# silvanmelchior/CBF-SSM

Measured on AMD Instinct MI355X. Metric: ELBO steps/sec, higher is better.
Workload: dtype f64; 1 GPU; C3-Sarcos train step: M=100 T=250 B=256/GPU S=20 dim_x=14 dim_u=7 dim_y=7 recog_len=16; mode=train, global_batch=256, seq_len=250, particles=20, parallelism=dp1

## Files before the change

cbf-ssm_amd/cbfssm/hip/lib.py:

```python
import ctypes as C
import os

_HERE = os.path.dirname(os.path.abspath(__file__))
LIB_PATH = os.environ.get('CBFSSM_HIP_LIB') or os.path.normpath(os.path.join(_HERE, '..', '..', 'lib', 'libcbfssm_hip.so'))

SCAL_SIGMA2, SCAL_LOGDET, SCAL_KLZ, SCAL_INFO, SCAL_COND, SCAL_JITTER, SCAL_COUNT = 0, 1, 2, 3, 4, 5, 16
GP_FORM_DENSE, GP_FORM_TRI = 0, 1
JITTER = 1e-8

SYMBOLS = (
    'cbfssm_last_error', 'cbfssm_version', 'cbfssm_gp_pack_layout', 'cbfssm_kmm_chol_f64', 'cbfssm_gp_prepare_f64',
    'cbfssm_gp_predict_f64', 'cbfssm_backward_pass_partials', 'cbfssm_backward_pass_f64',
    'cbfssm_forward_pass_partials', 'cbfssm_forward_pass_f64', 'cbfssm_loglik_moments_f64',
    'cbfssm_elbo_combine_f64', 'cbfssm_rev_workgroups', 'cbfssm_bwd_schedule', 'cbfssm_forward_pass_bwd_f64',
    'cbfssm_backward_pass_bwd_f64', 'cbfssm_reduce_partials_f64', 'cbfssm_gp_prepare2_f64', 'cbfssm_bwd_segments', 'cbfssm_forward_pass_bwd_ex_f64',
    'cbfssm_backward_pass_bwd_ex_f64', 'cbfssm_half_forward_pass_f64', 'cbfssm_half_forward_pass_bwd_f64',
    'cbfssm_saved_a2_elems', 'cbfssm_param_layout_init', 'cbfssm_constrain_f64', 'cbfssm_train_tail_work_elems',
    'cbfssm_train_tail_f64', 'cbfssm_train_tail_g_f64', 'cbfssm_train_tail_half_work_elems', 'cbfssm_train_tail_half_f64', 'cbfssm_gru_recog_param_elems', 'cbfssm_gru_recog_act_elems', 'cbfssm_gru_recog_f64', 'cbfssm_gru_recog_bwd_f64',
    'cbfssm_conv_recog_param_elems', 'cbfssm_conv_recog_f32', 'cbfssm_conv_recog_bwd_f32', 'cbfssm_adam_step_f64', 'cbfssm_loglik_partials', 'cbfssm_data_tail_f64', 'cbfssm_stash_contract_work_elems', 'cbfssm_stash_contract_f64',
    'cbfssm_cholesky_f64', 'cbfssm_rbf_k_f64', 'cbfssm_gp_predict_fullq_work_elems', 'cbfssm_gp_predict_fullq_f64',
    'cbfssm_pack_f32_elems', 'cbfssm_gp_pack_f32', 'cbfssm_gp_pack_bf16', 'cbfssm_gp_predict_f32', 'cbfssm_backward_pass_f32', 'cbfssm_forward_pass_f32',
    'cbfssm_saved_a2_f32_elems', 'cbfssm_half_forward_pass_f32', 'cbfssm_half_forward_pass_bwd_f32', 'cbfssm_rev32_slab_elems', 'cbfssm_normal_f64', 'cbfssm_philox4x32_10_u32', 'cbfssm_forward_pass_bwd_f32', 'cbfssm_backward_pass_bwd_f32',
    'cbfssm_input_adjoint_fwd_elems', 'cbfssm_input_adjoint_bwd_elems', 'cbfssm_input_adjoint_obs_elems',
    'cbfssm_forward_pass_bwd_in_f64', 'cbfssm_backward_pass_bwd_in_f64', 'cbfssm_input_grads_f64',
    'cbfssm_gp_predict_bwd_workgroups', 'cbfssm_gp_predict_bwd_work_elems', 'cbfssm_gp_predict_bwd_f64', 'cbfssm_gp_tail_f64',
    'cbfssm_gp_rollout_partials', 'cbfssm_gp_rollout_f64', 'cbfssm_gp_rollout_bwd_workgroups', 'cbfssm_gp_rollout_bwd_work_elems',
    'cbfssm_gp_rollout_bwd_f64',
    'cbfssm_gp_filter_partials', 'cbfssm_gp_filter_f64', 'cbfssm_gp_filter_bwd_workgroups', 'cbfssm_gp_filter_bwd_work_elems',
    'cbfssm_gp_filter_bwd_f64',
    'cbfssm_rigid_filter_partials', 'cbfssm_rigid_filter_f64', 'cbfssm_rigid_filter_bwd_f64',
    'cbfssm_gru_recog_bwd_in_f64', 'cbfssm_conv_recog_bwd_in_f32', 'cbfssm_half_forward_pass_bwd_in_f64',
    'cbfssm_half_input_grads_f64',
)


class ParamLayout(C.Structure):
    _fields_ = [('off', C.c_int64 * 12), ('total', C.c_int64)] + [(n, C.c_int32) for n in ('M', 'D', 'dim_x', 'dim_y')]


class PackLayout(C.Structure):
    _fields_ = [(n, C.c_int64) for n in ('total', 'Bp', 'Zp', 'cz', 'muA', 's2A', 'invl', 'scal', 'Kmm', 'L', 'Kinv',
                                          'Linvt', 'Zs', 'muB', 's2B', 'ZT', 'rev_slab', 'work', 'Wp', 'WTp')] + \
               [(n, C.c_int32) for n in ('M', 'D', 'Do', 'NBLK', 'DK', 'Mp', 'Dp', 'KS', 'JB', 'rev_stash', 'gp_form',
                                         'reserved')]


class Problem(C.Structure):
    _fields_ = [(n, C.c_int32) for n in ('B', 'S', 'T', 'dim_x', 'dim_u', 'dim_y', 'M', 'recog_len', 'condition',
                                          'half', 'group0', 'ngroups')] + [('k_factor', C.c_double)]


class RigidBody(C.Structure):
    _fields_ = [('mass_inv', C.c_double), ('inertia_inv', C.c_double * 3), ('gravity', C.c_double * 3), ('dt', C.c_double)]


class CbfssmHipError(RuntimeError):
    pass


_lib = None


def load():
    global _lib
    if _lib is not None:
        return _lib
    import torch
    if not os.path.exists(LIB_PATH):
        raise CbfssmHipError('HIP extension not built: %s is missing (run __graft_entry__.build() / make -C '
                             'cbf-ssm_amd/csrc). There is no fallback path.' % LIB_PATH)
    lib = C.CDLL(LIB_PATH)
    vp, ip, i64, dbl = C.c_void_p, C.c_int, C.c_int64, C.c_double
    lib.cbfssm_last_error.restype = C.c_char_p
    lib.cbfssm_last_error.argtypes = []
    lib.cbfssm_version.restype = ip
    lib.cbfssm_gp_pack_layout.argtypes = [ip, ip, ip, C.POINTER(PackLayout)]
    lib.cbfssm_kmm_chol_f64.argtypes = [ip, ip, vp, vp, vp, dbl, vp, vp, vp, vp, vp]
    lib.cbfssm_gp_prepare_f64.argtypes = [C.POINTER(PackLayout), vp, vp, vp, vp, vp, dbl, vp, vp]
    lib.cbfssm_gp_prepare2_f64.argtypes = ([C.POINTER(PackLayout)] + [vp] * 6) * 2 + [dbl, vp]
    lib.cbfssm_gp_predict_f64.argtypes = [C.POINTER(PackLayout), vp, vp, i64, vp, vp, vp]
    lib.cbfssm_backward_pass_partials.restype = i64
    lib.cbfssm_backward_pass_partials.argtypes = [C.POINTER(Problem)]
    lib.cbfssm_backward_pass_f64.argtypes = [C.POINTER(Problem), C.POINTER(PackLayout)] + [vp] * 12
    lib.cbfssm_forward_pass_partials.restype = i64
    lib.cbfssm_loglik_partials.restype = i64
    lib.cbfssm_loglik_partials.argtypes = [C.POINTER(Problem)]
    lib.cbfssm_param_layout_init.argtypes = [ip, ip, ip, ip, C.POINTER(ParamLayout)]
    lib.cbfssm_constrain_f64.argtypes = [C.POINTER(ParamLayout), vp, vp, vp]
    lib.cbfssm_train_tail_work_elems.restype = i64
    lib.cbfssm_train_tail_work_elems.argtypes = [C.POINTER(PackLayout), C.POINTER(PackLayout)]
    lib.cbfssm_train_tail_f64.argtypes = ([C.POINTER(ParamLayout), C.POINTER(PackLayout), vp, C.POINTER(PackLayout), vp, vp,
                                          vp, vp, i64, vp, vp, vp, vp, vp])
    lib.cbfssm_train_tail_g_f64.argtypes = ([C.POINTER(ParamLayout), C.POINTER(PackLayout), vp, C.POINTER(PackLayout), vp, vp,
                                            vp, vp, i64, ip, vp, vp, vp, vp, vp])
    lib.cbfssm_train_tail_half_work_elems.restype = i64
    lib.cbfssm_train_tail_half_work_elems.argtypes = [C.POINTER(PackLayout)]
    lib.cbfssm_train_tail_half_f64.argtypes = [C.POINTER(PackLayout), vp, vp, ip, vp, vp, i64, ip, ip, vp, vp, vp, vp, vp]
    lib.cbfssm_gru_recog_param_elems.restype = i64
    lib.cbfssm_gru_recog_param_elems.argtypes = [ip, ip, ip]
    lib.cbfssm_gru_recog_act_elems.restype = i64
    lib.cbfssm_gru_recog_act_elems.argtypes = [ip, ip]
    lib.cbfssm_gru_recog_f64.argtypes = [ip, ip, ip, ip, ip, ip, vp, vp, vp, vp, vp, vp]
    lib.cbfssm_gru_recog_bwd_f64.argtypes = [ip, ip, ip, ip, ip, ip, vp, vp, vp, vp, vp, vp, vp]
    lib.cbfssm_conv_recog_param_elems.restype = i64
    lib.cbfssm_conv_recog_param_elems.argtypes = [ip, ip, ip, ip]
    lib.cbfssm_conv_recog_f32.argtypes = [ip, ip, ip, ip, ip, ip, vp, vp, vp, vp, vp]
    lib.cbfssm_conv_recog_bwd_f32.argtypes = [ip, ip, ip, ip, ip, ip, vp, vp, vp, vp, vp, vp]
    lib.cbfssm_stash_contract_work_elems.restype = i64
    lib.cbfssm_stash_contract_work_elems.argtypes = [C.POINTER(PackLayout), i64]
    lib.cbfssm_stash_contract_f64.argtypes = [C.POINTER(PackLayout), vp, vp, i64, vp, vp, vp]
    lib.cbfssm_data_tail_f64.argtypes = [C.POINTER(Problem), vp, vp, vp, dbl, vp, vp]
    lib.cbfssm_adam_step_f64.argtypes = [i64, vp, vp, vp, vp, vp, dbl, dbl, dbl, dbl, vp]
    lib.cbfssm_saved_a2_elems.restype = i64
    lib.cbfssm_saved_a2_elems.argtypes = [C.POINTER(Problem), C.POINTER(PackLayout), ip]
    lib.cbfssm_forward_pass_partials.argtypes = [C.POINTER(Problem)]
    lib.cbfssm_forward_pass_f64.argtypes = [C.POINTER(Problem), C.POINTER(PackLayout)] + [vp] * 12
    lib.cbfssm_loglik_moments_f64.argtypes = [C.POINTER(Problem)] + [vp] * 9
    lib.cbfssm_elbo_combine_f64.argtypes = [C.POINTER(Problem), dbl, dbl, vp, i64, vp, i64, vp, i64, vp, vp, vp, vp]
    lib.cbfssm_rev_workgroups.restype = i64
    lib.cbfssm_rev_workgroups.argtypes = [C.POINTER(Problem), ip]
    lib.cbfssm_bwd_schedule.restype = ip
    lib.cbfssm_bwd_schedule.argtypes = [C.POINTER(Problem), ip] + [C.POINTER(C.c_int)] * 3
    lib.cbfssm_forward_pass_bwd_f64.argtypes = [C.POINTER(Problem), C.POINTER(PackLayout)] + [vp] * 10 + [dbl, vp, vp, vp]
    lib.cbfssm_backward_pass_bwd_f64.argtypes = [C.POINTER(Problem), C.POINTER(PackLayout)] + [vp] * 10 + [dbl, vp, vp]
    lib.cbfssm_bwd_segments.argtypes = [C.POINTER(Problem)]
    lib.cbfssm_forward_pass_bwd_ex_f64.argtypes = ([C.POINTER(Problem), C.POINTER(PackLayout)] + [vp] * 10 + [dbl, vp, vp, ip, ip, vp, vp, vp, i64, vp])
    lib.cbfssm_backward_pass_bwd_ex_f64.argtypes = ([C.POINTER(Problem), C.POINTER(PackLayout)] + [vp] * 10 + [dbl, vp, ip, ip, ip, vp, vp, i64, vp])
    lib.cbfssm_half_forward_pass_f64.argtypes = [C.POINTER(Problem), C.POINTER(PackLayout)] + [vp] * 12
    lib.cbfssm_half_forward_pass_bwd_f64.argtypes = ([C.POINTER(Problem), C.POINTER(PackLayout)] + [vp] * 9 + [dbl, vp, vp, ip, ip, vp, vp, vp, i64, vp])
    lib.cbfssm_reduce_partials_f64.argtypes = [vp, i64, i64, vp, vp]
    lib.cbfssm_cholesky_f64.argtypes = [ip, vp, dbl, vp, vp, vp, vp]
    lib.cbfssm_rbf_k_f64.argtypes = [ip, ip, ip, vp, vp, vp, vp, vp, vp]
    lib.cbfssm_gp_predict_fullq_work_elems.restype = i64
    lib.cbfssm_gp_predict_fullq_work_elems.argtypes = [C.POINTER(PackLayout), i64]
    lib.cbfssm_gp_predict_fullq_f64.argtypes = [C.POINTER(PackLayout), vp, vp, vp, i64, vp, vp, vp, vp]
    lib.cbfssm_pack_f32_elems.restype = i64
    lib.cbfssm_pack_f32_elems.argtypes = [C.POINTER(PackLayout)]
    lib.cbfssm_gp_pack_f32.argtypes = [C.POINTER(PackLayout), vp, vp, vp]
    lib.cbfssm_gp_pack_bf16.argtypes = [C.POINTER(PackLayout), vp, vp, vp]
    lib.cbfssm_gp_predict_f32.argtypes = [C.POINTER(PackLayout), vp, vp, i64, vp, vp, vp]
    lib.cbfssm_backward_pass_f32.argtypes = [C.POINTER(Problem), C.POINTER(PackLayout)] + [vp] * 12
    lib.cbfssm_forward_pass_f32.argtypes = [C.POINTER(Problem), C.POINTER(PackLayout)] + [vp] * 12
    lib.cbfssm_half_forward_pass_f32.argtypes = [C.POINTER(Problem), C.POINTER(PackLayout)] + [vp] * 12
    lib.cbfssm_half_forward_pass_bwd_f32.argtypes = [C.POINTER(Problem), C.POINTER(PackLayout)] + [vp] * 9 + [dbl, vp, vp, vp]
    lib.cbfssm_saved_a2_f32_elems.restype = i64
    lib.cbfssm_normal_f64.argtypes = [C.c_uint64, C.c_uint64, i64, vp, vp]
    lib.cbfssm_philox4x32_10_u32.argtypes = [C.c_uint64, C.c_uint64, i64, vp, vp]
    lib.cbfssm_saved_a2_f32_elems.argtypes = [C.POINTER(Problem), C.POINTER(PackLayout), ip]
    lib.cbfssm_rev32_slab_elems.restype = i64
    lib.cbfssm_rev32_slab_elems.argtypes = [C.POINTER(PackLayout)]
    lib.cbfssm_forward_pass_bwd_f32.argtypes = [C.POINTER(Problem), C.POINTER(PackLayout)] + [vp] * 10 + [dbl, vp, vp, vp]
    lib.cbfssm_backward_pass_bwd_f32.argtypes = [C.POINTER(Problem), C.POINTER(PackLayout)] + [vp] * 10 + [dbl, vp, vp]
    for name in ('cbfssm_input_adjoint_fwd_elems', 'cbfssm_input_adjoint_bwd_elems', 'cbfssm_input_adjoint_obs_elems'):
        getattr(lib, name).restype = i64
        getattr(lib, name).argtypes = [C.POINTER(Problem)]
    lib.cbfssm_forward_pass_bwd_in_f64.argtypes = ([C.POINTER(Problem), C.POINTER(PackLayout)] + [vp] * 10 + [dbl, vp, vp, ip, ip, vp, vp, vp, i64, vp, vp, vp])
    lib.cbfssm_backward_pass_bwd_in_f64.argtypes = ([C.POINTER(Problem), C.POINTER(PackLayout)] + [vp] * 10 + [dbl, vp, ip, ip, ip, vp, vp, i64, vp, vp])
    lib.cbfssm_input_grads_f64.argtypes = [C.POINTER(Problem), C.POINTER(PackLayout), vp, C.POINTER(PackLayout), vp] + [vp] * 6 + [dbl, vp, vp, vp]
    for name in ('cbfssm_gp_predict_bwd_workgroups', 'cbfssm_gp_predict_bwd_work_elems'):
        getattr(lib, name).restype = i64
        getattr(lib, name).argtypes = [C.POINTER(PackLayout), i64]
    lib.cbfssm_gp_predict_bwd_f64.argtypes = [C.POINTER(PackLayout), vp, vp, i64, vp, vp, vp, vp, vp, vp, vp]
    lib.cbfssm_gp_tail_f64.argtypes = [C.POINTER(PackLayout), vp, vp, vp, i64, dbl, vp, vp, vp, vp, vp]
    for name in ('cbfssm_gp_rollout_partials', 'cbfssm_gp_rollout_bwd_workgroups'):
        getattr(lib, name).restype = i64
        getattr(lib, name).argtypes = [C.POINTER(PackLayout), i64]
    lib.cbfssm_gp_rollout_bwd_work_elems.restype = i64
    lib.cbfssm_gp_rollout_bwd_work_elems.argtypes = [C.POINTER(PackLayout), i64, i64]
    lib.cbfssm_gp_rollout_f64.argtypes = [C.POINTER(PackLayout), vp, vp, vp, vp, vp, i64, i64, ip, vp, vp, vp, vp]
    lib.cbfssm_gp_rollout_bwd_f64.argtypes = [C.POINTER(PackLayout)] + [vp] * 8 + [i64, i64, ip] + [vp] * 6
    for name in ('cbfssm_gp_filter_partials', 'cbfssm_gp_filter_bwd_workgroups'):
        getattr(lib, name).restype = i64
        getattr(lib, name).argtypes = [C.POINTER(PackLayout), i64]
    lib.cbfssm_gp_filter_bwd_work_elems.restype = i64
    lib.cbfssm_gp_filter_bwd_work_elems.argtypes = [C.POINTER(PackLayout), i64, i64]
    lib.cbfssm_gp_filter_f64.argtypes = [C.POINTER(PackLayout)] + [vp] * 8 + [dbl, i64, i64, ip] + [vp] * 5
    lib.cbfssm_gp_filter_bwd_f64.argtypes = [C.POINTER(PackLayout)] + [vp] * 7 + [dbl] + [vp] * 5 + [i64, i64, ip] + [vp] * 7
    lib.cbfssm_rigid_filter_partials.restype = i64
    lib.cbfssm_rigid_filter_partials.argtypes = [i64]
    lib.cbfssm_rigid_filter_f64.argtypes = [C.POINTER(RigidBody)] + [vp] * 6 + [i64, i64] + [vp] * 3
    lib.cbfssm_rigid_filter_bwd_f64.argtypes = [C.POINTER(RigidBody)] + [vp] * 9 + [i64, i64] + [vp] * 5
    lib.cbfssm_gru_recog_bwd_in_f64.argtypes = [ip, ip, ip, ip, ip, ip, vp, vp, vp, vp, vp, vp, vp, vp]
    lib.cbfssm_conv_recog_bwd_in_f32.argtypes = [ip, ip, ip, ip, ip, ip, vp, vp, vp, vp, vp, vp, vp]
    lib.cbfssm_half_forward_pass_bwd_in_f64.argtypes = ([C.POINTER(Problem), C.POINTER(PackLayout)] + [vp] * 9 +
                                                        [dbl, vp, vp, ip, ip, vp, vp, vp, i64, vp, vp, vp])
    lib.cbfssm_half_input_grads_f64.argtypes = [C.POINTER(Problem), C.POINTER(PackLayout)] + [vp] * 8 + [ip, dbl, vp, vp, vp]
    for name in SYMBOLS:
        fn = getattr(lib, name)
        if name.endswith('_elems'):
            assert fn.restype is i64, name
            continue
        if fn.restype is C.c_int or name.endswith('_f64') or name.endswith('_f32') or name.endswith('_bf16') or name in ('cbfssm_gp_pack_layout', 'cbfssm_bwd_segments',
                                                                        'cbfssm_param_layout_init'):
            fn.restype = ip
    _lib = lib
    return lib


def param_layout(M, dim_x, dim_u, dim_y):
    pl = ParamLayout()
    check(load().cbfssm_param_layout_init(int(M), int(dim_x), int(dim_u), int(dim_y), C.byref(pl)), 'cbfssm_param_layout_init')
    return pl


def check(rc, what):
    if rc != 0:
        msg = load().cbfssm_last_error().decode('utf-8', 'replace')
        raise CbfssmHipError('%s failed (rc=%d): %s' % (what, rc, msg))


def rigid_body(mass_inv, inertia_inv, gravity, dt):
    rb = RigidBody()
    rb.mass_inv, rb.dt = float(mass_inv), float(dt)
# ... 18 lines not shown
```

cbf-ssm_amd/cbfssm/hip/ops.py:

```python
import ctypes as C
import os
import torch

from . import lib as _l


def _ptr(t):
    if t is None:
        return None
    assert t.is_cuda and t.dtype == torch.float64 and t.is_contiguous(), 'need contiguous float64 CUDA tensor'
    return C.c_void_p(t.data_ptr())


def _stream():
    return C.c_void_p(torch.cuda.current_stream().cuda_stream)


def _f64(t, device):
    return torch.as_tensor(t, dtype=torch.float64, device=device).contiguous()


F32_FORM_COND = 1e3


# ... 167 lines not shown


def as_btsd(x_tnd, B, S):
    T, N, d = x_tnd.shape
    return x_tnd.view(T, B, S, d).permute(1, 0, 2, 3)


def a2s_budget_bytes(device):
    cap = os.environ.get('CBFSSM_A2S_MAX_GB')
    if cap is not None:
        return float(cap) * 2 ** 30
    return 0.75 * torch.cuda.mem_get_info(torch.device(device))[0]


class TilePool:

    def __init__(self, device):
        self.device = torch.device(device)
        self.bufs = None
        self.retired = []
        self.budget = None
        self.log = []

    def get(self, n_f, n_b, reserve=0.0):
        import warnings
        if self.bufs is not None and self.bufs[0].numel() >= n_f and (n_b == 0 or (self.bufs[1] is not None and
                                                                                  self.bufs[1].numel() >= n_b)):
            return self.bufs[0][:max(n_f, 1)], (self.bufs[1][:max(n_b, 1)] if n_b else None)
        if self.budget is None:
            self.budget = a2s_budget_bytes(self.device)
        have = 0 if self.bufs is None else 8.0 * (self.bufs[0].numel() + (self.bufs[1].numel() if self.bufs[1] is not None else 0))
        need = 8.0 * (n_f + n_b)
        free_now = torch.cuda.mem_get_info(self.device)[0]
        held = float(self.bytes())
        if held + need > self.budget or need + reserve > 0.9 * free_now:
            msg = ('saved A2 tiles of this shape need %.2f GB, over the budget of %.2f GB (CBFSSM_A2S_MAX_GB): its adjoint '
                   'recomputes A2 (slower, same numbers)' % (need / 2 ** 30, self.budget / 2 ** 30))
            self.log.append(msg)
            warnings.warn(msg)
            return None, None
        if self.bufs is not None:
            msg = ('saved-A2 pool grows from %.2f to %.2f GB for a larger shape; the old buffers stay allocated for the '
                   'graphs captured on them' % (have / 2 ** 30, need / 2 ** 30))
            self.log.append(msg)
            warnings.warn(msg)
            self.retired.append(self.bufs)
        f = dict(dtype=torch.float64, device=self.device)
        self.bufs = (torch.zeros(max(n_f, 1), **f), torch.zeros(max(n_b, 1), **f) if n_b else None)
        return self.bufs[0][:max(n_f, 1)], (self.bufs[1][:max(n_b, 1)] if n_b else None)

    def bytes(self):
        tot = 0
        for pair in ([self.bufs] if self.bufs is not None else []) + self.retired:
            tot += 8 * (pair[0].numel() + (pair[1].numel() if pair[1] is not None else 0))
        return tot


class ElboWorkspace:

    def __init__(self, prob, device, keep_h=False, packs=None, pool=None):
        p = prob
        N, T = p.B * p.S, p.T
        dob = p.dim_x - p.dim_y
        f = dict(dtype=torch.float64, device=device)
        lib = _l.load()
        self.n_ent = int(lib.cbfssm_backward_pass_partials(C.byref(p)))
        self.n_kl = int(lib.cbfssm_forward_pass_partials(C.byref(p)))
        self.y2 = torch.zeros(T, N, dob, **f)
        self.h_all = torch.zeros(2, T, N, dob, **f) if keep_h else None
        self.fmv_b = torch.zeros(2, T, N, dob, 2, **f) if keep_h else None
        self.fmv_f = torch.zeros(max(T - 1, 0), N, p.dim_x, 2, **f) if keep_h else None
        self.a2s_f = self.a2s_b = None
        if keep_h and packs is not None:
            n_f = int(lib.cbfssm_saved_a2_elems(C.byref(p), C.byref(packs[0].layout), 0))
            n_b = int(lib.cbfssm_saved_a2_elems(C.byref(p), C.byref(packs[1].layout), 1)) if packs[1] is not None else 0
            if pool is None:
                pool = TilePool(device)
            reserve = 8.0 * T * N * (3 * p.dim_x + 8 * dob) + 2.0 * 2 ** 30
            self.a2s_f, self.a2s_b = pool.get(n_f, n_b, reserve)
        self.x = torch.zeros(T, N, p.dim_x, **f)
        self.ent_part = torch.zeros(self.n_ent, **f)
        self.kl_part = torch.zeros(self.n_kl, **f)
        self.ll_part = torch.zeros(int(lib.cbfssm_loglik_partials(C.byref(p))), **f)
        self.pred_mean = torch.zeros(p.B, T, p.dim_y, **f)
        self.pred_var = torch.zeros(p.B, T, p.dim_y, **f)
        self.int_mean = torch.zeros(p.B, T, p.dim_x, **f)
        self.int_var = torch.zeros(p.B, T, p.dim_x, **f)
        self.out = torch.zeros(8, **f)


def reduce_partials(gpart, slab, n, out, st):
    lib = _l.load()
    _l.check(lib.cbfssm_reduce_partials_f64(_ptr(gpart), slab, n, _ptr(out), st), 'cbfssm_reduce_partials_f64')


class TimeLoops:

    def __init__(self, prob, ws, pack_f, pack_b, var_x, var_y, u, y, eps_f, hid_b=None, eps_b=None, x0=None,
                 cL=0.0, cE=0.0, f32=False, bf16=False):
        self.prob, self.ws, self.pack_f, self.pack_b = prob, ws, pack_f, pack_b
        self.var_x, self.var_y, self.u, self.y, self.x0, self.eps_f, self.hid_b, self.eps_b = \
            var_x, var_y, u, y, x0, eps_f, hid_b, eps_b
        self.cL, self.cE, self.f32, self.bf16 = cL, cE, f32, bf16
        self.in_bufs = None

    def cast_f32(self):
        for pk in (self.pack_b, self.pack_f):
            if self.f32 and pk is not None:
                pk.pack_f32(self.bf16)

    def _gp(self, pack):
        return C.c_void_p(pack.buf32.data_ptr()) if self.f32 else _ptr(pack.buf)

    def _check(self, rc, name):
        _l.check(rc, 'cbfssm_%s_%s' % (name, 'f32' if self.f32 else 'f64'))

    def _fwd_args(self, q, *mid):
        ws = self.ws
        return ((C.byref(q), C.byref(self.pack_f.layout), self._gp(self.pack_f), _ptr(self.var_x), _ptr(self.var_y),
                 _ptr(self.u), _ptr(self.y)) + tuple(_ptr(t) for t in mid) +
                (_ptr(self.eps_f) if self.eps_f.numel() else None, _ptr(ws.x), _ptr(ws.fmv_f), _ptr(ws.a2s_f)))

    def _bwd_args(self, q):
        return (C.byref(q), C.byref(self.pack_b.layout), self._gp(self.pack_b), _ptr(self.var_x), _ptr(self.u),
                _ptr(self.y), _ptr(self.hid_b), _ptr(self.eps_b))

    def backward_pass(self, q, st):
        lib, ws = _l.load(), self.ws
        a = self._bwd_args(q) + (_ptr(ws.y2), _ptr(ws.h_all), _ptr(ws.fmv_b), _ptr(ws.a2s_b), _ptr(ws.ent_part), st)
        self._check(lib.cbfssm_backward_pass_f32(*a) if self.f32 else lib.cbfssm_backward_pass_f64(*a), 'backward_pass')

    def forward_pass(self, q, st):
        lib = _l.load()
        a = self._fwd_args(q, self.ws.y2) + (_ptr(self.ws.kl_part), st)
        self._check(lib.cbfssm_forward_pass_f32(*a) if self.f32 else lib.cbfssm_forward_pass_f64(*a), 'forward_pass')

    def forward_pass_bwd(self, q, st, chunk=None):
        lib, ws = _l.load(), self.ws
        a = self._fwd_args(q, ws.y2) + (self.cL, _ptr(ws.gy2), _ptr(ws.gpart_f))
        if self.in_bufs is not None:
            t_hi, t_lo, sa, sk, cols = chunk or (q.T - 2, 0, None, None, 0)
            _l.check(lib.cbfssm_forward_pass_bwd_in_f64(*a, t_hi, t_lo, _ptr(ws.gx_carry) if chunk else None, _ptr(sa), _ptr(sk),
                                                        cols, _ptr(self.in_bufs[0]), _ptr(self.in_bufs[2]), st),
                     'cbfssm_forward_pass_bwd_in_f64')
        elif chunk is None:
            self._check(lib.cbfssm_forward_pass_bwd_f32(*a, st) if self.f32 else lib.cbfssm_forward_pass_bwd_f64(*a, st),
                        'forward_pass_bwd')
        else:
            t_hi, t_lo, sa, sk, cols = chunk
            _l.check(lib.cbfssm_forward_pass_bwd_ex_f64(*a, t_hi, t_lo, _ptr(ws.gx_carry), _ptr(sa), _ptr(sk), cols, st),
                     'cbfssm_forward_pass_bwd_ex_f64')

    def backward_pass_bwd(self, q, st, chunk=None):
        lib, ws = _l.load(), self.ws
        a = self._bwd_args(q) + (_ptr(ws.h_all), _ptr(ws.fmv_b), _ptr(ws.a2s_b), _ptr(ws.gy2), self.cE, _ptr(ws.gpart_b))
        if self.in_bufs is not None:
            if chunk is None:
                nchunk = 0
                chunk = (0, int(lib.cbfssm_bwd_segments(C.byref(q))), None, None, 0)
            else:
                nchunk = 1
            seg0, seg1, sa, sk, cols = chunk
            _l.check(lib.cbfssm_backward_pass_bwd_in_f64(*a, seg0, seg1, nchunk, _ptr(sa), _ptr(sk), cols,
                                                         _ptr(self.in_bufs[1]), st), 'cbfssm_backward_pass_bwd_in_f64')
        elif chunk is None:
            self._check(lib.cbfssm_backward_pass_bwd_f32(*a, st) if self.f32 else lib.cbfssm_backward_pass_bwd_f64(*a, st),
                        'backward_pass_bwd')
        else:
            seg0, seg1, sa, sk, cols = chunk
            _l.check(lib.cbfssm_backward_pass_bwd_ex_f64(*a, seg0, seg1, 1, _ptr(sa), _ptr(sk), cols, st),
                     'cbfssm_backward_pass_bwd_ex_f64')

    def input_grads(self, grad_u, grad_y, st):
        ws, (gin_f, gin_b, gyo) = self.ws, self.in_bufs
        _l.check(_l.load().cbfssm_input_grads_f64(C.byref(self.prob), C.byref(self.pack_f.layout), _ptr(self.pack_f.buf),
                                                  C.byref(self.pack_b.layout), _ptr(self.pack_b.buf), _ptr(self.var_y),
                                                  _ptr(self.y), _ptr(ws.x), _ptr(gin_f), _ptr(gin_b), _ptr(gyo), self.cL,
                                                  _ptr(grad_u), _ptr(grad_y), st), 'cbfssm_input_grads_f64')

    def half_forward_pass(self, q, st):
        lib = _l.load()
        a = self._fwd_args(q, self.x0) + (_ptr(self.ws.kl_part), st)
        self._check(lib.cbfssm_half_forward_pass_f32(*a) if self.f32 else lib.cbfssm_half_forward_pass_f64(*a),
                    'half_forward_pass')

    def half_forward_pass_bwd(self, q, st, chunk=None):
        lib, ws = _l.load(), self.ws
        a = self._fwd_args(q) + (self.cL, _ptr(ws.gx0), _ptr(ws.gpart_f))
        if self.f32:
            rc = lib.cbfssm_half_forward_pass_bwd_f32(*a, st)
        else:
            t_hi, t_lo, sa, sk, cols = chunk or (q.T - 2, 0, None, None, 0)
            r = (t_hi, t_lo, _ptr(ws.gx_carry) if chunk else None, _ptr(sa), _ptr(sk), cols)
            if self.in_bufs is not None:
                _l.check(lib.cbfssm_half_forward_pass_bwd_in_f64(*a, *r, _ptr(self.in_bufs[0]), _ptr(self.in_bufs[2]), st),
                         'cbfssm_half_forward_pass_bwd_in_f64')
                return
            rc = lib.cbfssm_half_forward_pass_bwd_f64(*a, *r, st)
        self._check(rc, 'half_forward_pass_bwd')

    def half_input_grads(self, gx0, gwin, recog_len, grad_u, grad_y, st):
        ws, (gin_f, _, gyo) = self.ws, self.in_bufs
        _l.check(_l.load().cbfssm_half_input_grads_f64(C.byref(self.prob), C.byref(self.pack_f.layout), _ptr(self.pack_f.buf),
                                                       _ptr(self.var_y), _ptr(self.y), _ptr(ws.x), _ptr(gin_f), _ptr(gyo),
                                                       _ptr(gx0), _ptr(gwin), int(recog_len), self.cL, _ptr(grad_u),
                                                       _ptr(grad_y), st), 'cbfssm_half_input_grads_f64')

    def elbo_tail(self, lf0, lf1, st, kl_pack=None):
        lib, ws, pb = _l.load(), self.ws, C.byref(self.prob)
        _l.check(lib.cbfssm_loglik_moments_f64(pb, _ptr(self.var_y), _ptr(self.y), _ptr(ws.x), _ptr(ws.ll_part),
                                               _ptr(ws.pred_mean), _ptr(ws.pred_var), _ptr(ws.int_mean),
                                               _ptr(ws.int_var), st), 'cbfssm_loglik_moments_f64')
        b = self.pack_b is not None
        _l.check(lib.cbfssm_elbo_combine_f64(pb, float(lf0), float(lf1), _ptr(ws.ll_part), ws.ll_part.numel(),
                                             _ptr(ws.kl_part), ws.kl_part.numel(), _ptr(ws.ent_part) if b else None,
                                             ws.ent_part.numel() if b else 0, _ptr((kl_pack or self.pack_f).scal),
                                             _ptr(self.pack_b.scal) if b else None, _ptr(ws.out), st),
                 'cbfssm_elbo_combine_f64')


def elbo_forward(lp, loss_factors):
    prob, st = lp.prob, _stream()
    N = prob.B * prob.S
    assert lp.u.shape == (prob.B, prob.T, prob.dim_u) and lp.y.shape == (prob.B, prob.T, prob.dim_y)
    assert lp.hid_b.numel() == 2 * prob.T * N and lp.eps_b.numel() == 2 * prob.T * N
    assert lp.eps_f.numel() == (prob.T - 1) * N
    lp.cast_f32()
    lp.backward_pass(prob, st)
    lp.forward_pass(prob, st)
    lp.elbo_tail(loss_factors[0], loss_factors[1], st)
    return lp.ws


def tf_forward(x):
    return torch.nn.functional.softplus(x, beta=1.0, threshold=1e9) + 1e-10


class HipElbo:

    def __init__(self, config, device, dtype='float64'):
        self.config = config
        self.device = torch.device(device)
        assert dtype in ('float64', 'float32', 'bfloat16')
        self.f32 = dtype in ('float32', 'bfloat16')
        self.bf16 = dtype == 'bfloat16'
        self.dim_u, self.dim_y, self.dim_x = config['ds'].dim_u, config['ds'].dim_y, config['dim_x']
        self.M, self.S = config['ind_pnt_num'], config['samples']
        D = self.dim_x + self.dim_u
        mode = gp_form_mode(config) if not self.f32 else gp_form_mode_f32(config, self.bf16)
        self.pack_f = GPPack(self.M, D, self.dim_x, self.device, mode)
        self.pack_b = GPPack(self.M, D, self.dim_x - self.dim_y, self.device, mode)
        if self.f32:
            self.pack_f.cond_threshold = self.pack_b.cond_threshold = min(self.pack_f.cond_threshold, F32_FORM_COND)
        self._ws = {}

    def gp_form(self):
        return self.pack_f.gp_form() + '/' + self.pack_b.gp_form()

    def prepare(self, params):
        p = {k: _f64(v, self.device) for k, v in params.items()}
        args = [(p[g + '.zeta_pos'], tf_forward(p[g + '.lengthscales_unc']), tf_forward(p[g + '.variance_unc']),
                 p[g + '.zeta_mean'], tf_forward(p[g + '.zeta_var_unc'])) for g in 'fb']
        prepare_pair(self.pack_f, args[0], self.pack_b, args[1])
        for pk in (self.pack_f, self.pack_b):
            pk.update_form(blocking=True)
        self.var_x = tf_forward(p['var_x_unc']).contiguous()
        self.var_y = tf_forward(p['var_y_unc']).contiguous()

    def problem(self, B, T, condition):
        c = self.config
        return _l.make_problem(B, self.S, T, self.dim_x, self.dim_u, self.dim_y, self.M, c['recog_len'],
                               c['k_factor'], condition)

    def run(self, u, y, noise, condition=True, keep_h=False):
        u, y = _f64(u, self.device), _f64(y, self.device)
        B, T = u.shape[0], u.shape[1]
        prob = self.problem(B, T, condition)
        key = (B, T, keep_h)
        if key not in self._ws:
            self._ws[key] = ElboWorkspace(prob, self.device, keep_h)
        ws = self._ws[key]
        hid_b, eps_b, eps_f = (_f64(noise[k], self.device) for k in ('hid_b', 'eps_b', 'eps_f'))
        return elbo_forward(TimeLoops(prob, ws, self.pack_f, self.pack_b, self.var_x, self.var_y, u, y, eps_f, hid_b, eps_b,
                                      f32=self.f32, bf16=self.bf16), self.config['loss_factors'])


class NoisePipeline:

    def __init__(self, device, generator=None, with_backward=True):
        self.device = torch.device(device)
        self.gen = generator
        self.with_backward = with_backward
        self.stream = torch.cuda.Stream(device=self.device)
        self._bufs = {}
        self._ready = {}
        self.use_lib = not os.environ.get('CBFSSM_TORCH_NOISE')
        self.seed = int(generator.initial_seed()) & (2 ** 64 - 1) if generator is not None else int.from_bytes(os.urandom(8), 'little')
        self.offset = 0

    def _numel(self, T, N):
        return (4 * T * N if self.with_backward else 0) + (T - 1) * N

    def _fill(self, key, idx):
        buf = self._bufs[key][idx]
        cur = torch.cuda.current_stream(self.device)
        self.stream.wait_stream(cur)
        with torch.cuda.stream(self.stream):
            if self.use_lib:
                rc = _l.load().cbfssm_normal_f64(self.seed, self.offset, buf.numel(), _ptr(buf),
                                                 C.c_void_p(self.stream.cuda_stream))
                _l.check(rc, 'cbfssm_normal_f64')
                self.offset += buf.numel()
            else:
# ... 20 lines not shown
```

cbf-ssm_amd/cbfssm/hip/train.py:

```python
import ctypes as C
import math
import os
import torch

from . import lib as _l
from . import ops
from .ops import _ptr, _stream, _f64, tf_forward, GPPack
from .dist_utils import all_reduce_sum

PARAM_NAMES = (
    'f.zeta_pos', 'f.zeta_mean', 'f.zeta_var_unc', 'f.variance_unc', 'f.lengthscales_unc',
    'b.zeta_pos', 'b.zeta_mean', 'b.zeta_var_unc', 'b.variance_unc', 'b.lengthscales_unc',
    'var_x_unc', 'var_y_unc',
)
LOG2PI = math.log(2.0 * math.pi)


class FlatDict(dict):
    flat = None


def _flat_views(flat, pl, dim_u):
    M, D, dx, dy = pl.M, pl.D, pl.dim_x, pl.dim_y
    shapes = []
# ... 197 lines not shown
        else:
            loss = out[6].clone()
            terms = {'loglik': out[0], 'kl_x': out[1], 'entropy': out[2], 'kl_z_f': out[3], 'kl_z_b': out[4],
                     'info': out[7]}
        self.last_ws = ws
        return loss, terms, ws

    def _prepare(self, params, u, y, condition):
        cfg = self.config
        u, y = _f64(u, self.device), _f64(y, self.device)
        prob = _l.make_problem(u.shape[0], self.S, u.shape[1], self.dim_x, self.dim_u, self.dim_y, self.M,
                               cfg['recog_len'], cfg['k_factor'], condition)
        pflat = self._flat(params)
        p, c = self._constrained_flat(pflat)
        ops.prepare_pair(self.pack_f, (p['f.zeta_pos'], c['f.ls'], c['f.var'], p['f.zeta_mean'], c['f.zvar']),
                         self.pack_b, (p['b.zeta_pos'], c['b.ls'], c['b.var'], p['b.zeta_mean'], c['b.zvar']))
        return u, y, prob, pflat, p, c

    def _workspace(self, prob):
        key = (prob.B, prob.T)
        if key not in self._ws:
            ws = ops.ElboWorkspace(prob, self.device, keep_h=True, packs=None if self.f32 else (self.pack_f, self.pack_b),
                                   pool=self.tile_pool)
            lib = _l.load()
            n_f = int(lib.cbfssm_rev_workgroups(C.byref(prob), 0))
            n_b = int(lib.cbfssm_rev_workgroups(C.byref(prob), 1))
            f = dict(dtype=torch.float64, device=self.device)
            ws.gy2 = torch.zeros_like(ws.y2)
            if self.f32:
                if not os.environ.get('CBFSSM_F32_NO_TILES'):
                    na_f = (int(lib.cbfssm_saved_a2_f32_elems(C.byref(prob), C.byref(self.pack_f.layout), 0)) + 1) // 2
                    na_b = (int(lib.cbfssm_saved_a2_f32_elems(C.byref(prob), C.byref(self.pack_b.layout), 1)) + 1) // 2
                    assert na_f >= 0 and na_b > 0, 'record count'
                    reserve = 8.0 * prob.T * prob.B * prob.S * (3 * prob.dim_x + 8 * self.dob) + 2.0 * 2 ** 30
                    ws.a2s_f, ws.a2s_b = self.tile_pool.get(max(na_f, 1), na_b, reserve)
                sf, sb = self.slab32_f, self.slab32_b
            else:
                if self.stash:
                    n_b = 2 * n_f
                    ws.gx_carry = torch.zeros(prob.B * prob.S, prob.dim_x, **f)
                sf, sb = self.slab_f, self.slab_b
            ws.gpart_f = torch.zeros((n_f + 32) * sf, **f)
            ws.gpart_b = torch.zeros((n_b + 32) * sb, **f)
            ws.n_f, ws.n_b = n_f, n_b
            self._ws[key] = ws
        return self._ws[key]

    def loss_and_grads(self, params, u, y, noise, condition=True, weight=1.0, local=False, input_grads=False):
        s = self._grads_local(params, u, y, noise, condition, input_grads=input_grads)
        if not local:
            self._grads_collective(s, weight)
        return self._grads_finish(s)

    def _grads_collective(self, s, weight=1.0):
        if self.dist is not None:
            if weight != 1.0:
                self.red.mul_(float(weight))
            all_reduce_sum(self.red, self.dist)

    def _need_input_grads(self):
        need_input_grads(self.f32, self.dist)

    def _input_buffers(self, prob, ws):
        if getattr(ws, 'in_bufs', None) is None:
            lib = _l.load()
            f = dict(dtype=torch.float64, device=self.device)
            n = [int(fn(C.byref(prob))) for fn in (lib.cbfssm_input_adjoint_fwd_elems, lib.cbfssm_input_adjoint_bwd_elems,
                                                   lib.cbfssm_input_adjoint_obs_elems)]
            assert min(n) >= 0, n
            ws.in_bufs = tuple(torch.zeros(max(k, 1), **f) for k in n)
            ws.grad_u = torch.zeros(prob.B, prob.T, prob.dim_u, **f)
            ws.grad_y = torch.zeros(prob.B, prob.T, prob.dim_y, **f)
        return ws.in_bufs

    def _grads_local(self, params, u, y, noise, condition=True, input_grads=False):
        self._need_adjoint()
        if input_grads:
            self._need_input_grads()
        u, y, prob, pflat, p, c = self._prepare(params, u, y, condition)
        self.last_ws = ws = self._workspace(prob)
        lp = self._loops(prob, ws, c, u, y, noise)
        if input_grads:
            lp.in_bufs = self._input_buffers(prob, ws)
        self._elbo_forward(lp)
        if self.stash and not self.f32:
            gB_f, gB_b = self._adjoint_stash(lp, self.red)
        else:
            gB_f, gB_b = self._adjoint(lp, self.red)
        if input_grads:
            lp.input_grads(ws.grad_u, ws.grad_y, _stream())
        sf, sb = self.slab_f, self.slab_b
        tail = self.red[sf + sb:sf + sb + self.ntail]
        _l.check(_l.load().cbfssm_data_tail_f64(C.byref(prob), _ptr(c['var_y']), _ptr(ws.ll_part), _ptr(ws.out), lp.cL,
                                          _ptr(tail), _stream()), 'cbfssm_data_tail_f64')
        return dict(ws=ws, p=p, c=c, pflat=pflat, gB_f=gB_f, gB_b=gB_b, cL=lp.cL, cE=lp.cE, input_grads=bool(input_grads))

    def _grads_finish(self, s):
        lib = _l.load()
        st = _stream()
        ws, p, c, pflat, gB_f, gB_b, cL, cE = (s[k] for k in ('ws', 'p', 'c', 'pflat', 'gB_f', 'gB_b', 'cL', 'cE'))
        red = self.red
        sf, sb = self.slab_f, self.slab_b
        tail = red[sf + sb:sf + sb + self.ntail]
        loglik, kl_x, entropy = tail[0], tail[1], tail[2]
        kl_z_f, kl_z_b = self.pack_f.scal[_l.SCAL_KLZ], self.pack_b.scal[_l.SCAL_KLZ]
        if self.dist is not None:
            loss = -(loglik * cL - kl_x * cL + entropy * cE - kl_z_f - kl_z_b)
        else:
            loss = ws.out[6].clone()
        terms = {'loglik': loglik, 'kl_x': kl_x, 'entropy': entropy, 'kl_z_f': kl_z_f, 'kl_z_b': kl_z_b,
                 'info': ws.out[7]}
        if self.fused_tail:
            rc = lib.cbfssm_train_tail_g_f64(C.byref(self.pl), C.byref(self.pack_f.layout), _ptr(self.pack_f.buf),
                                             C.byref(self.pack_b.layout), _ptr(self.pack_b.buf), _ptr(red), _ptr(gB_f),
                                             _ptr(gB_b), 0, g_mode(self.f32, self.pack_f.layout), _ptr(pflat),
                                             _ptr(self.cflat), _ptr(self.tail_work), _ptr(self.gflat), st)
            _l.check(rc, 'cbfssm_train_tail_g_f64')
            grads = _flat_views(self.gflat, self.pl, self.dim_u)
        else:
            grads = self._grads_tensor_library(p, c, red, tail, gB_f, gB_b)
        if s.get('input_grads'):
            grads['u'], grads['y'] = ws.grad_u, ws.grad_y
        return loss, grads, terms

    def _grads_tensor_library(self, p, c, red, tail, gB_f, gB_b):
        dev = self.device
        sf, sb = self.slab_f, self.slab_b
        grads = {}
        gvx = torch.zeros(self.dim_x, dtype=torch.float64, device=dev)
        gvy = torch.zeros(self.dim_x, dtype=torch.float64, device=dev)
        if self.f32:
            gB_f, gB_b = kgk_image(self.pack_f, red[:sf], gB_f), kgk_image(self.pack_b, red[sf:sf + sb], gB_b)
        for g, pack, slab, Do, gBx in (('f', self.pack_f, red[:sf], self.dim_x, gB_f),
                                       ('b', self.pack_b, red[sf:sf + sb], self.dob, gB_b)):
            gz, gmu, gs2, gvar, gls, small = _gp_adjoint(pack, slab, p[g + '.zeta_pos'], c[g + '.ls'], c[g + '.var'],
                                                         p[g + '.zeta_mean'], c[g + '.zvar'], Do, not self.stash, gBx)
            grads.update(gp_unc_grads(g + '.', p, gz, gmu, gs2, gvar, gls))
            gvx[:Do] += small[0:Do]
            if g == 'f':
                gvy += small[16:16 + self.dim_x]
        gvy[:self.dim_y] += tail[3:]
        grads['var_x_unc'] = gvx * torch.sigmoid(p['var_x_unc'])
        grads['var_y_unc'] = gvy * torch.sigmoid(p['var_y_unc'])
        return grads

    def _split(self, prob, adjoint=True):
        if (self.stash and adjoint) or os.environ.get('CBFSSM_NO_SPLIT'):
            return None
        groups = (prob.B * prob.S + 15) // 16
        force = os.environ.get('CBFSSM_SPLIT_MAIN')
        if force:
            return (int(force), groups - int(force)) if 0 < int(force) < groups else None
        ncu = torch.cuda.get_device_properties(self.device).multi_processor_count
        if groups <= ncu or groups % ncu == 0:
            return None
        main = (groups // ncu) * ncu
        return main, groups - main

    def _sub_problem(self, prob, g0, ng):
        q = _l.Problem()
        C.memmove(C.byref(q), C.byref(prob), C.sizeof(_l.Problem))
        q.group0, q.ngroups = int(g0), int(ng)
        return q

    def _side_stream(self):
        if getattr(self, '_s1', None) is None:
            self._s1 = torch.cuda.Stream(device=self.device)
        return self._s1

    def _loops(self, prob, ws, c, u, y, noise):
        hid_b, eps_b, eps_f = (_f64(noise[k], self.device) for k in ('hid_b', 'eps_b', 'eps_f'))
        lf = self.config['loss_factors']
        return ops.TimeLoops(prob, ws, self.pack_f, self.pack_b, c['var_x'], c['var_y'], u, y, eps_f, hid_b, eps_b,
                             cL=float(lf[0]) / self.S, cE=float(lf[1]) / self.S, f32=self.f32)

    def _two_streams(self, prob, split):
        main, rest = split
        s0, s1 = torch.cuda.current_stream(), self._side_stream()
        return (self._sub_problem(prob, 0, main), self._sub_problem(prob, main, rest), s0, s1,
                C.c_void_p(s0.cuda_stream), C.c_void_p(s1.cuda_stream))

    def _elbo_forward(self, lp):
        lf = self.config['loss_factors']
        split = self._split(lp.prob, adjoint=False)
        if split is None:
            ops.elbo_forward(lp, lf)
            return
        p_main, p_rest, s0, s1, st0, st1 = self._two_streams(lp.prob, split)
        lp.cast_f32()
        e0 = torch.cuda.Event()
        e0.record(s0)
        lp.backward_pass(p_rest, st0)
        lp.forward_pass(p_rest, st0)
        s1.wait_event(e0)
        lp.backward_pass(p_main, st1)
        e1 = torch.cuda.Event()
        e1.record(s1)
        s0.wait_event(e1)
        lp.forward_pass(p_main, st0)
        lp.elbo_tail(lf[0], lf[1], st0)

    def _adjoint(self, lp, red):
        ws, st = lp.ws, _stream()
        sf, sb = self.slab_f, self.slab_b
        split = self._split(lp.prob, adjoint=False)
        if split is None:
            lp.forward_pass_bwd(lp.prob, st)
            lp.backward_pass_bwd(lp.prob, st)
        else:
            p_main, p_rest, s0, s1, st0, st1 = self._two_streams(lp.prob, split)
            lp.forward_pass_bwd(p_main, st0)
            e2 = torch.cuda.Event()
            e2.record(s0)
            lp.forward_pass_bwd(p_rest, st0)
            s1.wait_event(e2)
            lp.backward_pass_bwd(p_main, st1)
            e3 = torch.cuda.Event()
            e3.record(s1)
            lp.backward_pass_bwd(p_rest, st0)
            s0.wait_event(e3)
        if not self.repack32:
            assert not self.f32 or (self.slab32_f, self.slab32_b) == (sf, sb)
            ops.reduce_partials(ws.gpart_f, sf, ws.n_f, red[:sf], st)
            ops.reduce_partials(ws.gpart_b, sb, ws.n_b, red[sf:sf + sb], st)
            return None, None
        if self._tmp32 is None:
            self._tmp32 = torch.zeros(self.slab32_f + self.slab32_b, dtype=torch.float64, device=self.device)
        tf, tb = self._tmp32[:self.slab32_f], self._tmp32[self.slab32_f:]
        ops.reduce_partials(ws.gpart_f, self.slab32_f, ws.n_f, tf, st)
        ops.reduce_partials(ws.gpart_b, self.slab32_b, ws.n_b, tb, st)
        o = self.nred
        img_f, img_b = red[o:o + self.nimg_f], red[o + self.nimg_f:o + self.nimg_f + self.nimg_b]
        repack_f32(tf, red[:sf], img_f, self.pack_f.layout.NBLK)
        repack_f32(tb, red[sf:sf + sb], img_b, self.pack_b.layout.NBLK)
        return img_f, img_b

    def _adjoint_stash(self, lp, red):
        prob, ws = lp.prob, lp.ws
        dev = self.device
        f = dict(dtype=torch.float64, device=dev)
        Mp = self.pack_f.layout.Mp
        T, N = prob.T, prob.B * prob.S
        groups = (N + 15) // 16
        R = prob.recog_len
        P = 2 * R
        cols_f = max(groups * 16, self.stash_bytes // (4 * Mp * 8))
        cols_b = max(groups * 16 * 2 * P, self.stash_bytes // (4 * Mp * 8))
        if self._stash_buf is None or self._stash_buf[0].numel() < Mp * cols_f or self._stash_buf[2].numel() < Mp * cols_b:
            self._stash_buf = (torch.zeros(Mp * cols_f, **f), torch.zeros(Mp * cols_f, **f),
                               torch.zeros(Mp * cols_b, **f), torch.zeros(Mp * cols_b, **f))
        sa_f, sk_f, sa_b, sk_b = self._stash_buf
        sf, sb = self.slab_f, self.slab_b
        nseg = int(_l.load().cbfssm_bwd_segments(C.byref(prob)))
        per_b = max(1, cols_b // (groups * 2 * P * 16))
        prof = getattr(self, '_prof', None)
        overlap = not os.environ.get('CBFSSM_NO_SPLIT') and prof is None
        s0 = torch.cuda.current_stream()
        s1 = self._side_stream() if overlap else s0
        st0, st1 = C.c_void_p(s0.cuda_stream), C.c_void_p(s1.cuda_stream)
        red[:sf + sb].zero_()
        tmp_f, tmp_b = torch.zeros(max(sf, 1), **f), torch.zeros(max(sb, 1), **f)
        if getattr(self, '_contract', None) is None:
            o = self.nred
            self._contract = (StashContract(self.pack_f, dev, red[o:o + self.nimg_f]),
                              StashContract(self.pack_b, dev, red[o + self.nimg_f:o + self.nimg_f + self.nimg_b]))
        con_f, con_b = self._contract
        con_f.image.zero_()
        con_b.image.zero_()
        if overlap:
            s1.wait_stream(s0)

        def rfwd(t_hi, t_lo):
            per = max(1, cols_f // (groups * 16))
            while True:
                lo = max(t_lo, t_hi - per + 1)
                cols = groups * max(0, t_hi - lo + 1) * 16
                _timed(prof, 'forward_pass_adjoint', s0,
                       lambda: lp.forward_pass_bwd(prob, st0, (t_hi, lo, sa_f, sk_f, cols)))
                ev = torch.cuda.Event()
                ev.record(s0)

                def red_f():
                    ops.reduce_partials(ws.gpart_f, sf, groups, tmp_f[:sf], st0)
                    red[:sf] += tmp_f[:sf]
                _timed(prof, 'reductions', s0, red_f)
                if cols:
                    _timed(prof, 'stash_contraction', s0, lambda: con_f.add(sa_f, sk_f, cols, st0))
                if lo <= t_lo or t_hi < 0:
                    return ev
                t_hi = lo - 1

        def rbwd(seg0, seg1):
            cols = groups * 2 * (seg1 - seg0) * P * 16
            with torch.cuda.stream(s1):
                _timed(prof, 'backward_pass_adjoint', s1,
                       lambda: lp.backward_pass_bwd(prob, st1, (seg0, seg1, sa_b, sk_b, cols)))

                def red_b():
                    ops.reduce_partials(ws.gpart_b, sb, 2 * groups, tmp_b[:sb], st1)
                    red[sf:sf + sb] += tmp_b[:sb]
                _timed(prof, 'reductions', s1, red_b)
                _timed(prof, 'stash_contraction', s1, lambda: con_b.add(sa_b, sk_b, cols, st1))

        t_hi = T - 2
        seg1 = nseg
        done_all = (t_hi < 0)
        if done_all:
            rfwd(-1, 0)
# ... 66 lines not shown
class TFAdam:

    def __init__(self, params, lr, beta1=0.9, beta2=0.999, eps=1e-8):
        self.names = list(params.keys())
        sizes = [params[k].numel() for k in self.names]
        dev = params[self.names[0]].device
        self.flat = torch.cat([params[k].reshape(-1) for k in self.names]).to(torch.float64).contiguous()
        self.m = torch.zeros_like(self.flat)
        self.v = torch.zeros_like(self.flat)
        self.gflat = torch.zeros_like(self.flat)
        self.views, self.gviews = FlatDict(), {}
        self.views.flat = self.flat
        o = 0
        for k, n in zip(self.names, sizes):
            self.views[k] = self.flat[o:o + n].view(params[k].shape)
            self.gviews[k] = self.gflat[o:o + n].view(params[k].shape)
            o += n
        self.lr, self.b1, self.b2, self.eps = float(lr), beta1, beta2, eps
        self.t_dev = torch.zeros(1, dtype=torch.float64, device=dev)
        self._t = 0

    @property
    def t(self):
        return self._t

    @t.setter
    def t(self, value):
        self._t = int(value)
        self.t_dev.fill_(float(value))

    def step(self, grads):
        gflat = getattr(grads, 'flat', None)
        if gflat is not None and gflat.is_cuda and gflat.numel() == self.flat.numel():
            rc = _l.load().cbfssm_adam_step_f64(self.flat.numel(), _ptr(self.flat), _ptr(gflat), _ptr(self.m),
                                                _ptr(self.v), _ptr(self.t_dev), self.lr, self.b1, self.b2, self.eps,
                                                _stream())
            _l.check(rc, 'cbfssm_adam_step_f64')
            self._t += 1
            return
        for k in self.names:
            self.gviews[k].copy_(grads[k])
        self.t = self._t + 1
        g = self.gflat
        self.m.mul_(self.b1).add_(g, alpha=1 - self.b1)
        self.v.mul_(self.b2).addcmul_(g, g, value=1 - self.b2)
        lr_t = self.lr * math.sqrt(1 - self.b2 ** self.t) / (1 - self.b1 ** self.t)
        self.flat.addcdiv_(self.m, self.v.sqrt().add_(self.eps), value=-lr_t)

    def step_device(self, grads):
        for k in self.names:
            self.gviews[k].copy_(grads[k])
        self.t_dev.add_(1.0)
        self._t += 1
        g = self.gflat
        self.m.mul_(self.b1).add_(g, alpha=1 - self.b1)
        self.v.mul_(self.b2).addcmul_(g, g, value=1 - self.b2)
        b1t = torch.pow(torch.full_like(self.t_dev, self.b1), self.t_dev)
        b2t = torch.pow(torch.full_like(self.t_dev, self.b2), self.t_dev)
        lr_t = self.lr * torch.sqrt(1.0 - b2t) / (1.0 - b1t)
        self.flat.sub_(lr_t * self.m / (self.v.sqrt() + self.eps))

    def state_dict(self):
        return {'flat': self.flat.clone(), 'm': self.m.clone(), 'v': self.v.clone(), 't': self.t, 'names': self.names}

    def load_state_dict(self, sd):
        self.flat.copy_(sd['flat'])
        self.m.copy_(sd['m'])
        self.v.copy_(sd['v'])
        self.t = int(sd['t'])


class HipTrainStep:

    def __init__(self, config, params, device, dist=None, graph=None, engine=None, opt=None, dtype='float64'):
        if engine is None:
            engine = HipElboGrad(config, device, dist, dtype=dtype)
            opt = TFAdam({k: _f64(params[k], device).clone() for k in PARAM_NAMES}, config['learning_rate'])
        self.engine, self.opt = engine, opt
        self.params = self.opt.views
        if graph is None:
            graph = config.get('hip_graph', os.environ.get('CBFSSM_HIP_GRAPH', '1') != '0')
        self.use_graph = bool(graph) and not self.engine.stash
        self._graphs = {}
        self.last_ws = None

    def step(self, u, y, noise, condition=True, weight=1.0, local=False):
        if self.use_graph and not local:
            return self._graph_step(u, y, noise, condition, weight)
        loss, grads, terms = self.engine.loss_and_grads(self.params, u, y, noise, condition, weight=weight, local=local)
        self.opt.step(grads)
        self.last_terms = terms
        self.last_ws = self.engine.last_ws
        return loss

    def _graph_step(self, u, y, noise, condition, weight=1.0):
        dev = self.engine.device
        u, y = _f64(u, dev), _f64(y, dev)
        key = (tuple(u.shape), tuple(y.shape), bool(condition), self.engine.gp_forms())
        g = self._graphs.get(key)
        names = ('hid_b', 'eps_b', 'eps_f')
        if g is None:
            g = {'u': u.clone(), 'y': y.clone(), 'noise': {k: _f64(noise[k], dev).clone() for k in names}}
            cur = torch.cuda.current_stream(dev)
            side = torch.cuda.Stream(device=dev)
            side.wait_stream(cur)
            with torch.cuda.stream(side):
                self.engine.loss_and_grads(self.params, g['u'], g['y'], g['noise'], condition, local=True)
            cur.wait_stream(side)
            eng = self.engine
            front = None
            t_before = self.opt._t
            mode = 'global' if eng.dist is None else 'thread_local'
            try:
                if eng.dist is not None:
                    torch.cuda.synchronize(dev)
                    front = torch.cuda.CUDAGraph()
                    with torch.cuda.graph(front, capture_error_mode=mode):
                        state = eng._grads_local(self.params, g['u'], g['y'], g['noise'], condition)
                graph = torch.cuda.CUDAGraph()
                with torch.cuda.graph(graph, capture_error_mode=mode):
                    if front is None:
                        state = eng._grads_local(self.params, g['u'], g['y'], g['noise'], condition)
                    loss, grads, terms = eng._grads_finish(state)
                    if getattr(grads, 'flat', None) is not None:
                        self.opt.step(grads)
                    else:
                        self.opt.step_device(grads)
                    self.opt._t -= 1
            except RuntimeError as e:
                if eng.dist is None:
                    raise
                import warnings
                warnings.warn('HIP graph capture failed on this rank (%s): continuing with eager launches' % e)
                torch.cuda.synchronize(dev)
                self.opt._t = t_before
                self.use_graph = False
                return self.step(u, y, noise, condition, weight=weight)
            g.update(graph=graph, front=front, state=state, loss=loss, terms=terms, ws=state['ws'])
            self._graphs[key] = g
        else:
            g['u'].copy_(u)
            g['y'].copy_(y)
            for k in names:
                g['noise'][k].copy_(_f64(noise[k], dev))
        if g['front'] is not None:
            g['front'].replay()
            self.engine._grads_collective(g['state'], weight)
        g['graph'].replay()
        self.opt._t += 1
        self.last_terms = g['terms']
        self.last_ws = g['ws']
        return g['loss'].clone()
```

cbf-ssm_amd/csrc/cbfssm_api.hip:

```cpp
#include <hip/hip_runtime.h>
#include <cmath>
#include <cstdio>
#include <cstring>
#include <cstdarg>
#include <cstdlib>
#include <algorithm>
#include <map>
#include <mutex>
#include <vector>
#include "../../include/cbfssm_hip.h"
#include "cbfssm_inst.hpp"
#include "cbfssm_adjoint_inst.hpp"

CBF_FOR_EACH_NBLK(CBF_DECLARE)
CBF_FOR_EACH_REV_NBLK(CBF_REV_DECLARE)
CBF_FOR_EACH_REV_NBLK(CBF_REVIN_DECLARE)

namespace cbfssm {

static thread_local char g_err[512] = "";
static double* g_dbg = nullptr;

int fail(int code, const char* fmt, ...)
{
// ... 477 lines not shown
            hipError_t e = hipFuncSetAttribute(reinterpret_cast<const void*>(prepare_kernel<false>),
                                               hipFuncAttributeMaxDynamicSharedMemorySize, int(pl));
            if (e != hipSuccess) return fail(-int(e) - 1000, "prepare: %s", hipGetErrorString(e));
        }
        hipLaunchKernelGGL(prepare_kernel<false>, dim3(n), dim3(PREP_NT), pl, st, aa);
    }
    return check_launch("gp_prepare");
}

struct LlArgs {
    int B, S, T, dim_x, dim_y;
    const double* var_y;
    const double* y;
    const double* x;
    double* ll_part;
    double* pred_mean;
    double* pred_var;
    double* int_mean;
    double* int_var;
};

__global__ void loglik_moments_kernel(LlArgs a)
{
    __shared__ double sh[256];
    const int64_t idx = int64_t(blockIdx.x) * blockDim.x + threadIdx.x;
    const int64_t total = int64_t(a.B) * a.T * a.dim_x;
    double ll = 0.0;
    if (idx < total) {
        const int d = int(idx % a.dim_x);
        const int64_t tb = idx / a.dim_x;
        const int b = int(tb % a.B), t = int(tb / a.B);
        const int64_t bt = int64_t(b) * a.T + t;
        const int64_t N = int64_t(a.B) * a.S;
        const double* xp = a.x + (int64_t(t) * N + int64_t(b) * a.S) * a.dim_x + d;
        const double x0 = xp[0];
        double s1 = 0.0, s2 = 0.0;
        constexpr int CH = 19;
        int s = 1;
        for (; s + CH <= a.S; s += CH) {
            double v[CH];
#pragma unroll
            for (int j = 0; j < CH; ++j) v[j] = xp[int64_t(s + j) * a.dim_x];
#pragma unroll
            for (int j = 0; j < CH; ++j) {
                const double dv = v[j] - x0;
                s1 += dv;
                s2 += dv * dv;
            }
        }
#pragma unroll 8
        for (; s < a.S; ++s) {
            const double dv = xp[int64_t(s) * a.dim_x] - x0;
            s1 += dv;
            s2 += dv * dv;
        }
        const double m1 = s1 / a.S;
        const double mean = x0 + m1;
        const double ss = fmax(s2 - s1 * m1, 0.0);
        const double var = ss / a.S;
        if (a.int_mean) { a.int_mean[bt * a.dim_x + d] = mean; a.int_var[bt * a.dim_x + d] = var; }
        if (d < a.dim_y) {
            const double vy = a.var_y[d];
            const int64_t o = bt * a.dim_y + d;
            a.pred_mean[o] = mean;
            a.pred_var[o] = var + vy;
            const double yo = a.y[o];
            const double dm = yo - mean;
            const double sq = ss + a.S * dm * dm;
            ll = -0.5 * (sq / vy + a.S * (1.8378770664093454836 + log(vy)));
        }
    }
    sh[threadIdx.x] = ll;
    __syncthreads();
    if (int(threadIdx.x) < a.dim_y) {
        const int d = threadIdx.x;
        const int base = int((int64_t(blockIdx.x) * 256) % a.dim_x);
        double s = 0.0;
        for (int k = (d - base + a.dim_x) % a.dim_x; k < 256; k += a.dim_x) s += sh[k];
        a.ll_part[int64_t(blockIdx.x) * a.dim_y + d] = s;
    }
}

struct CombineArgs {
    const double* ll; int64_t n_ll;
    const double* kl; int64_t n_kl;
    const double* ent; int64_t n_ent;
    const double* scal_f;
    const double* scal_b;
    double lambda0, lambda1, inv_s;
    double* out;
};

__global__ __launch_bounds__(1024) void combine_kernel(CombineArgs a)
{
    __shared__ double red[16];
    const int tid = threadIdx.x;
    double s0 = 0.0, s1 = 0.0, s2 = 0.0;
    for (int64_t i = tid; i < a.n_ll; i += 1024) s0 += a.ll[i];
    for (int64_t i = tid; i < a.n_kl; i += 1024) s1 += a.kl[i];
    for (int64_t i = tid; i < a.n_ent; i += 1024) s2 += a.ent[i];
    const double loglik = block_sum(s0, red, tid, 1024);
    const double kl_x = block_sum(s1, red, tid, 1024);
    const double entropy = block_sum(s2, red, tid, 1024);
    if (tid == 0) {
        const double klf = a.scal_f[CBFSSM_SCAL_KLZ], klb = a.scal_b ? a.scal_b[CBFSSM_SCAL_KLZ] : 0.0;
        const double elbo = loglik * a.lambda0 * a.inv_s - kl_x * a.lambda0 * a.inv_s + entropy * a.lambda1 * a.inv_s
                            - klf - klb;
        a.out[0] = loglik; a.out[1] = kl_x; a.out[2] = entropy; a.out[3] = klf; a.out[4] = klb;
        a.out[5] = elbo; a.out[6] = -elbo;
        a.out[7] = fmax(a.scal_f[CBFSSM_SCAL_INFO], a.scal_b ? a.scal_b[CBFSSM_SCAL_INFO] : 0.0);
    }
}

#define RSPLIT 32
__global__ void reduce_partials_stage1(const double* gpart, int64_t slab, int nwg, double* tmp)
{
    const int64_t i = int64_t(blockIdx.x) * blockDim.x + threadIdx.x;
    if (i >= slab) return;
    const int part = blockIdx.y;
    const int per = (nwg + RSPLIT - 1) / RSPLIT;
    const int k0 = part * per, k1 = min(nwg, k0 + per);
    double s = 0.0;
    for (int k = k0; k < k1; ++k) s += gpart[int64_t(k) * slab + i];
    tmp[int64_t(part) * slab + i] = s;
}

__global__ void reduce_partials_stage2(const double* tmp, int64_t slab, double* out)
{
    const int64_t i = int64_t(blockIdx.x) * blockDim.x + threadIdx.x;
    if (i >= slab) return;
    double s = 0.0;
#pragma unroll
    for (int k = 0; k < RSPLIT; ++k) s += tmp[int64_t(k) * slab + i];
    out[i] = s;
}

struct InGradArgs {
    int B, S, T, dim_x, dim_u, dim_y;
    const double* gin_f;
    const double* gin_b;
    const double* gyo;
    const double* invl_f;
    const double* invl_b;
    const double* x;
    const double* y;
    const double* var_y;
    double cL;
    double* gu;
    double* gy;
};

__global__ void input_grads_kernel(InGradArgs a)
{
    const int64_t nu = int64_t(a.B) * a.T * a.dim_u, ny = int64_t(a.B) * a.T * a.dim_y;
    const int64_t i = int64_t(blockIdx.x) * blockDim.x + threadIdx.x;
    if (i >= nu + ny) return;
    const int64_t N = int64_t(a.B) * a.S;
    const int naux = a.dim_u + a.dim_y, dob = a.dim_x - a.dim_y;
    const bool is_u = i < nu;
    const int nd = is_u ? a.dim_u : a.dim_y;
    const int64_t e = is_u ? i : i - nu;
    const int k = int(e % nd);
    const int t = int((e / nd) % a.T);
    const int b = int(e / (int64_t(nd) * a.T));
    const int ja = is_u ? k : a.dim_u + k;
    const double* p0 = a.gin_b + ((int64_t(0) * a.T + t) * naux + ja) * N + int64_t(b) * a.S;
    const double* p1 = a.gin_b + ((int64_t(1) * a.T + t) * naux + ja) * N + int64_t(b) * a.S;
    double s0 = 0.0, s1 = 0.0;
    for (int s = 0; s < a.S; ++s) { s0 += p0[s]; s1 += p1[s]; }
    double r = a.invl_b[dob + ja] * (s0 + s1);
    if (is_u) {
        if (t < a.T - 1) {
            const double* pf = a.gin_f + (int64_t(t) * a.dim_u + k) * N + int64_t(b) * a.S;
            double sf = 0.0;
            for (int s = 0; s < a.S; ++s) sf += pf[s];
            r += a.invl_f[a.dim_x + k] * sf;
        }
        a.gu[e] = r;
    } else {
        const double* po = a.gyo + (int64_t(t) * a.dim_y + k) * N + int64_t(b) * a.S;
        const double* px = a.x + (int64_t(t) * N + int64_t(b) * a.S) * a.dim_x + k;
        const double yv = a.y[e];
        double so = 0.0, sl = 0.0;
        for (int s = 0; s < a.S; ++s) {
// ... 403 lines not shown
    PredictArgs a;
    a.pk = pack_ptrs(L, pack); a.X = X; a.npts = npts; a.D = L->D; a.Do = L->Do; a.fmean = fmean; a.fvar = fvar;
    a.tri = (L->gp_form == CBFSSM_GP_FORM_TRI);
    a.a2o = work;
    int rc = dispatch_predict(L->NBLK, L->DK, a, (hipStream_t)stream);
    if (rc) return fail(rc, "gp_predict launch failed (NBLK=%d DK=%d rc=%d)", L->NBLK, L->DK, rc);
    const size_t lds = size_t(16) * L->NBLK * 16 * sizeof(double);
    if (lds > 48 * 1024) {
        hipError_t e = hipFuncSetAttribute(reinterpret_cast<const void*>(fullq_kernel),
                                           hipFuncAttributeMaxDynamicSharedMemorySize, int(lds));
        if (e != hipSuccess) return fail(-int(e) - 1000, "fullq: %s", hipGetErrorString(e));
    }
    hipLaunchKernelGGL(fullq_kernel, dim3(unsigned((npts + 15) / 16), unsigned(L->Do)), dim3(256), lds, (hipStream_t)stream,
                       (const double*)work, q_sqrt, L->M, L->NBLK, L->Do, npts, fvar);
    return check_launch("gp_predict_fullq");
}

int64_t cbfssm_backward_pass_partials(const cbfssm_problem* p)
{
    if (!p || p->recog_len < 1) return -1;
    int n0, n1;
    bwd_segments(p, &n0, &n1);
    const int64_t groups = (int64_t(p->B) * p->S + 15) / 16;
    return groups * (n0 + n1);
}

static int save_k(const cbfssm_pack_layout* L);

int cbfssm_backward_pass_f64(const cbfssm_problem* p, const cbfssm_pack_layout* L, const double* pack_b,
                             const double* var_x, const double* u, const double* y, const double* hid_b,
                             const double* eps_b, double* y2, double* h_all, double* fmv_b, double* a2s_b,
                             double* ent_part, void* stream)
{
    int rc = check_problem(p, L, p ? p->dim_x - p->dim_y : 0);
    if (rc) return rc;
    if (p->dim_x - p->dim_y < 1) return fail(-1, "backward pass needs dim_x > dim_y (use CBFSSMHALF otherwise)");
    if (!pack_b || !var_x || !u || !y || !hid_b || !eps_b || !y2 || !ent_part) return fail(-1, "null pointer");
    PassArgs a;
    memset(&a, 0, sizeof(a));
    a.pk = pack_ptrs(L, pack_b);
    a.N = p->B * p->S; a.S = p->S; a.T = p->T; a.B = p->B;
    a.dim_x = p->dim_x; a.dim_u = p->dim_u; a.dim_y = p->dim_y; a.Do = p->dim_x - p->dim_y; a.D = L->D;
    a.recog_len = p->recog_len; a.condition = p->condition; a.k_factor = p->k_factor;
    a.var_x = var_x; a.u = u; a.y = y; a.eps = eps_b; a.hid = hid_b; a.y2_out = y2; a.h_all = h_all;
    a.part_out = ent_part;
    a.dbg = g_dbg;
    a.fmv = fmv_b;
    a.a2s = a2s_b;
    a.ksave = save_k(L);
    int n0, n1;
    bwd_segments(p, &n0, &n1);
    a.nseg0 = n0;
    a.tri = (L->gp_form == CBFSSM_GP_FORM_TRI);
    const int nc = a.tri ? 1 : pass_nc(p, MODE_BWD);
    int g0, ng, gt;
    rc = group_range(p, nc, &g0, &ng, &gt);
    if (rc) return rc;
    a.group0 = g0; a.gtotal = gt;
    dim3 grid(unsigned(ng), unsigned(n0 + n1));
    rc = dispatch_pass(L->NBLK, L->DK, MODE_BWD, a, grid, nc, (hipStream_t)stream);
    if (rc) return fail(rc, "backward_pass launch failed (NBLK=%d DK=%d rc=%d)", L->NBLK, L->DK, rc);
    return 0;
}

static int save_k(const cbfssm_pack_layout* L) { return (L->NBLK <= 7 && !getenv("CBFSSM_NO_SAVE_K")) ? 1 : 0; }

int64_t cbfssm_saved_a2_elems(const cbfssm_problem* p, const cbfssm_pack_layout* L, int backward)
{
    if (!p || !L) return -1;
    const int64_t g16 = (int64_t(p->B) * p->S + 15) / 16;
    const int64_t slots = backward ? 2 * int64_t(p->T) : (p->T > 1 ? p->T - 1 : 0);
    return slots * g16 * saved_tile_stride(L->NBLK, save_k(L));
}

int64_t cbfssm_forward_pass_partials(const cbfssm_problem* p)
{
    if (!p) return -1;
    return (int64_t(p->B) * p->S + 15) / 16;
}

static int forward_pass_impl(const cbfssm_problem* p, const cbfssm_pack_layout* L, const double* pack_f,
                             const double* var_x, const double* var_y, const double* u, const double* y,
                             const double* y2, const double* x0, const double* eps_f, double* x, double* fmv_f,
                             double* a2s_f, double* kl_part, void* stream)
{
    int rc = check_problem(p, L, p ? p->dim_x : 0);
    if (rc) return rc;
    if (!pack_f || !var_x || !var_y || !u || !y || !x || !kl_part) return fail(-1, "null pointer");
    if (p->half ? !x0 : (p->dim_x > p->dim_y && !y2)) return fail(-1, p->half ? "x0 is null" : "y2 is null");
    if (p->T > 1 && !eps_f) return fail(-1, "eps_f is null");
    PassArgs a;
    memset(&a, 0, sizeof(a));
    a.pk = pack_ptrs(L, pack_f);
    a.N = p->B * p->S; a.S = p->S; a.T = p->T; a.B = p->B;
    a.dim_x = p->dim_x; a.dim_u = p->dim_u; a.dim_y = p->dim_y; a.Do = p->dim_x; a.D = L->D;
    a.recog_len = p->recog_len; a.condition = p->condition; a.k_factor = p->k_factor;
    a.var_x = var_x; a.var_y = var_y; a.u = u; a.y = y; a.eps = eps_f; a.y2_in = y2; a.x_out = x;
    a.part_out = kl_part;
    a.dbg = g_dbg;
    a.half = p->half; a.x0 = x0;
    a.fmv = fmv_f;
    a.a2s = a2s_f;
    a.ksave = save_k(L);
    a.tri = (L->gp_form == CBFSSM_GP_FORM_TRI);
    const int nc = a.tri ? 1 : pass_nc(p, MODE_FWD);
    int g0, ng, gt;
    rc = group_range(p, nc, &g0, &ng, &gt);
    if (rc) return rc;
    a.group0 = g0; a.gtotal = gt;
    dim3 grid(unsigned(ng), 1);
    rc = dispatch_pass(L->NBLK, L->DK, MODE_FWD, a, grid, nc, (hipStream_t)stream);
    if (rc) return fail(rc, "forward_pass launch failed (NBLK=%d DK=%d rc=%d)", L->NBLK, L->DK, rc);
    return 0;
}

int cbfssm_forward_pass_f64(const cbfssm_problem* p, const cbfssm_pack_layout* L, const double* pack_f,
                            const double* var_x, const double* var_y, const double* u, const double* y,
                            const double* y2, const double* eps_f, double* x, double* fmv_f, double* a2s_f,
                            double* kl_part, void* stream)
{
    if (p && p->half) return fail(-1, "problem->half is set: use cbfssm_half_forward_pass_f64");
    return forward_pass_impl(p, L, pack_f, var_x, var_y, u, y, y2, nullptr, eps_f, x, fmv_f, a2s_f, kl_part, stream);
}

int cbfssm_half_forward_pass_f64(const cbfssm_problem* p, const cbfssm_pack_layout* L, const double* pack_f,
                                 const double* var_x, const double* var_y, const double* u, const double* y,
                                 const double* x0, const double* eps_f, double* x, double* fmv_f, double* a2s_f,
                                 double* kl_part, void* stream)
{
    if (!p || !p->half) return fail(-1, "problem->half must be 1");
    return forward_pass_impl(p, L, pack_f, var_x, var_y, u, y, nullptr, x0, eps_f, x, fmv_f, a2s_f, kl_part, stream);
}

int cbfssm_loglik_moments_f64(const cbfssm_problem* p, const double* var_y, const double* y, const double* x,
                              double* ll_part, double* pred_mean, double* pred_var, double* int_mean,
                              double* int_var, void* stream)
{
    if (!p || !var_y || !y || !x || !ll_part || !pred_mean || !pred_var) return fail(-1, "null pointer");
    if ((int_mean == nullptr) != (int_var == nullptr)) return fail(-1, "int_mean/int_var must both be given");
    LlArgs a;
    a.B = p->B; a.S = p->S; a.T = p->T; a.dim_x = p->dim_x; a.dim_y = p->dim_y;
    a.var_y = var_y; a.y = y; a.x = x; a.ll_part = ll_part; a.pred_mean = pred_mean; a.pred_var = pred_var;
    a.int_mean = int_mean; a.int_var = int_var;
    const int64_t total = int64_t(p->B) * p->T * p->dim_x;
    const int64_t nblk = (total + 255) / 256;
    hipLaunchKernelGGL(loglik_moments_kernel, dim3(unsigned(nblk)), dim3(256), 0, (hipStream_t)stream, a);
    return check_launch("loglik_moments");
}

int64_t cbfssm_loglik_partials(const cbfssm_problem* p)
{
    if (!p) return -1;
    return (int64_t(p->B) * p->T * p->dim_x + 255) / 256 * p->dim_y;
}

int cbfssm_elbo_combine_f64(const cbfssm_problem* p, double lambda0, double lambda1, const double* ll_part,
                            int64_t n_ll, const double* kl_part, int64_t n_kl, const double* ent_part, int64_t n_ent,
                            const double* scal_f, const double* scal_b, double* out, void* stream)
{
    if (!p || !scal_f || !out) return fail(-1, "null pointer");
    CombineArgs a;
    a.ll = ll_part; a.n_ll = ll_part ? n_ll : 0; a.kl = kl_part; a.n_kl = kl_part ? n_kl : 0;
    a.ent = ent_part; a.n_ent = ent_part ? n_ent : 0;
    a.scal_f = scal_f; a.scal_b = scal_b; a.lambda0 = lambda0; a.lambda1 = lambda1; a.inv_s = 1.0 / p->S;
    a.out = out;
    hipLaunchKernelGGL(combine_kernel, dim3(1), dim3(1024), 0, (hipStream_t)stream, a);
    return check_launch("elbo_combine");
}

constexpr int SCHED_UNITS = 256;
constexpr int SCHED_PER_RUN = 16;
constexpr int SCHED_PROLOGUE = 2;

struct SchedEntry { int run, t_begin, nsteps; };

static bool sched_table(int T, int R, int m, std::vector<SchedEntry>& out)
{
    const int P = 2 * R;
    out.clear();
    for (int run = 0; run < 2; ++run) {
        const int start = run * R;
        int rem = (T > start) ? (T - start + P - 1) / P : 0, pos = 0, cnt = 0;
        while (rem > 0) {
            const int c = std::min(m, std::max(1, rem / 2));
            const int tb = start + P * pos, te = std::min(T, start + P * (pos + c));
            out.push_back({run, tb, te - tb});
            pos += c; rem -= c;
            if (++cnt > SCHED_PER_RUN) return false;
        }
    }
    std::stable_sort(out.begin(), out.end(), [](const SchedEntry& x, const SchedEntry& y) { return x.nsteps > y.nsteps; });
    return true;
}

static int64_t sched_makespan(const std::vector<SchedEntry>& tab, int64_t groups)
{
    std::map<int64_t, int64_t> slots;
    slots[0] = SCHED_UNITS;
    for (const SchedEntry& e : tab) {
        int64_t left = groups;
        while (left > 0) {
            auto it = slots.begin();
            const int64_t t = it->first, take = std::min(left, it->second);
            if ((it->second -= take) == 0) slots.erase(it);
            slots[t + e.nsteps + SCHED_PROLOGUE] += take;
            left -= take;
        }
    }
    return slots.rbegin()->first;
}

static void bwd_schedule(int T, int R, int64_t n, std::vector<SchedEntry>& best)
{
    static std::mutex mu;
    static int cT = -1, cR = -1;
    static int64_t cn = -1;
    static std::vector<SchedEntry> cached;
    std::lock_guard<std::mutex> lock(mu);
    if (T != cT || R != cR || n != cn) {
        const int64_t groups = (n + 15) / 16;
        const int P = 2 * R;
        std::vector<SchedEntry> tab;
        int64_t best_t = -1;
        cached.clear();
        for (int m = std::max(1, (T + P - 1) / P); m >= 1; --m) {
            if (!sched_table(T, R, m, tab)) break;
            const int64_t t = sched_makespan(tab, groups);
            if (best_t < 0 || t < best_t) { best_t = t; cached = tab; }
        }
        cT = T; cR = R; cn = n;
    }
    best = cached;
}

static int bwd_total_segments(const cbfssm_problem* p)
{
    return (p->T - 1 + p->recog_len) / (2 * p->recog_len) + 1;
}

int cbfssm_bwd_schedule(const cbfssm_problem* p, int cap, int* run, int* t_begin, int* nsteps)
{
    if (!p || p->recog_len < 1 || p->T < 1 || p->B < 1 || p->S < 1) return fail(-1, "bad problem");
    std::vector<SchedEntry> tab;
    bwd_schedule(p->T, p->recog_len, int64_t(p->B) * p->S, tab);
    const int n = int(tab.size());
    if (run || t_begin || nsteps) {
        if (!run || !t_begin || !nsteps || cap < n) return fail(-1, "schedule has %d entries (cap %d)", n, cap);
        for (int i = 0; i < n; ++i) { run[i] = tab[i].run; t_begin[i] = tab[i].t_begin; nsteps[i] = tab[i].nsteps; }
    }
    return n;
// ... 330 lines not shown
```

cbf-ssm_amd/csrc/cbfssm_kernels.hpp:

```cpp
#pragma once
#include <hip/hip_runtime.h>
#include <stdint.h>
#include <type_traits>

namespace cbfssm {

typedef double d4 __attribute__((ext_vector_type(4)));

#define CBF_MFMA(a, b, c) __builtin_amdgcn_mfma_f64_16x16x4f64((a), (b), (c), 0, 0, 0)

__device__ __forceinline__ double fast_rcp(double x)
{
    double r = __builtin_amdgcn_rcp(x);
    r = fma(r, fma(-x, r, 1.0), r);
    return fma(r, fma(-x, r, 1.0), r);
}
__device__ __forceinline__ double fast_rsqrt(double x)
{
    double y = __builtin_amdgcn_rsq(x);
    const double hx = 0.5 * x;
    y = fma(y, fma(-hx * y, y, 0.5), y);
    return fma(y, fma(-hx * y, y, 0.5), y);
}

// ... 197 lines not shown
        "v_mfma_f64_16x16x4_f64 %[c01], v[150:151], v[166:167], %[c01]\n\t"
        "v_mfma_f64_16x16x4_f64 %[c11], v[158:159], v[166:167], %[c11]\n\t"
        "s_branch 4f\n\t"
        "3:\n"
        "s_waitcnt vmcnt(0) lgkmcnt(0)\n\t"
        "v_mfma_f64_16x16x4_f64 %[c00], v[120:121], v[136:137], %[c00]\n\t"
        "v_mfma_f64_16x16x4_f64 %[c10], v[128:129], v[136:137], %[c10]\n\t"
        "v_mfma_f64_16x16x4_f64 %[c01], v[122:123], v[138:139], %[c01]\n\t"
        "v_mfma_f64_16x16x4_f64 %[c11], v[130:131], v[138:139], %[c11]\n\t"
        "v_mfma_f64_16x16x4_f64 %[c00], v[124:125], v[140:141], %[c00]\n\t"
        "v_mfma_f64_16x16x4_f64 %[c10], v[132:133], v[140:141], %[c10]\n\t"
        "v_mfma_f64_16x16x4_f64 %[c01], v[126:127], v[142:143], %[c01]\n\t"
        "v_mfma_f64_16x16x4_f64 %[c11], v[134:135], v[142:143], %[c11]\n\t"
        "4:\n"
        "s_nop 15\n\t"
        "s_nop 2\n\t"
        : [c00] "+v"(c00), [c01] "+v"(c01), [c10] "+v"(c10), [c11] "+v"(c11), [pa0] "+v"(pa0), [pa1] "+v"(pa1),
          [pb] "+v"(ldsb), [n] "+s"(ngrp)
        : [step] "s"(step), [bs0] "n"(0 * BSTRIDE), [bs1] "n"(1 * BSTRIDE), [bs2] "n"(2 * BSTRIDE), [bs3] "n"(3 * BSTRIDE),
          [bs4] "n"(4 * BSTRIDE), [bs5] "n"(5 * BSTRIDE), [bs6] "n"(6 * BSTRIDE), [bs7] "n"(7 * BSTRIDE),
          [bs8] "n"(8 * BSTRIDE)
        : "scc", "v120", "v121", "v122", "v123", "v124", "v125", "v126", "v127", "v128", "v129", "v130", "v131", "v132", "v133", "v134", "v135", "v136", "v137", "v138", "v139", "v140", "v141", "v142", "v143", "v144", "v145", "v146", "v147", "v148", "v149", "v150", "v151", "v152", "v153", "v154", "v155", "v156", "v157", "v158", "v159", "v160", "v161", "v162", "v163", "v164", "v165", "v166", "v167");
}

struct PackPtrs {
    const double* Bp;
    const double* Zp;
    const double* cz;
    const double* muA;
    const double* s2A;
    const double* invl;
    const double* scal;
    int KSr;
    const double* Wp;
    const double* WTp;
};

typedef __attribute__((address_space(3))) int lds_int;
__device__ __forceinline__ void flag_release(int* f, int v)
{
    __hip_atomic_store((lds_int*)f, v, __ATOMIC_RELEASE, __HIP_MEMORY_SCOPE_WORKGROUP);
}
#define CBF_FLAG_TIMEOUT_SLOT 96
__device__ __forceinline__ void flag_wait(int* flags, int idx, int v)
{
    int spins = 0;
    while (__hip_atomic_load((lds_int*)(flags + idx), __ATOMIC_ACQUIRE, __HIP_MEMORY_SCOPE_WORKGROUP) < v) {
        __builtin_amdgcn_s_sleep(1);
        if (++spins > (1 << 22)) {
            __hip_atomic_store((lds_int*)(flags + CBF_FLAG_TIMEOUT_SLOT), 1, __ATOMIC_RELAXED, __HIP_MEMORY_SCOPE_WORKGROUP);
            break;
        }
    }
}

struct PassArgs {
    PackPtrs pk;
    int N, S, T, B;
    int dim_x, dim_u, dim_y;
    int Do;
    int D;
    int recog_len, condition;
    double k_factor;
    const double* var_x;
    const double* var_y;
    const double* u;
    const double* y;
    const double* eps;
    const double* hid;
    const double* y2_in;
    double* y2_out;
    double* h_all;
    double* x_out;
    double* part_out;
    int nseg0;
    double* dbg;
    int half;
    const double* x0;
    int group0, gtotal;
    double* a2s;
    double* fmv;
    int tri;
    int ksave;
};

__device__ __forceinline__ int bwd_segment(int y, int n0, int ny, int& run, int& k, bool& dead)
{
    const int n1 = ny - n0, w1 = max(0, n1 - 2);
    dead = false;
    if (y < n0 - 1) { run = 0; k = y + 1; }
    else if (y < n0 - 1 + w1) { run = 1; k = y - (n0 - 1) + 2; }
    else if (y == n0 - 1 + w1) { run = 0; k = n0; }
    else if (y == ny - 1) { run = 1; k = 1; dead = true; }
    else { run = 1; k = n1; }
    return run == 0 ? k - 1 : n0 + k - 1;
}

__host__ __device__ constexpr int saved_tile_stride(int nblk, int ksave) { return nblk * 256 * (ksave ? 2 : 1); }

struct PredictArgs {
    PackPtrs pk;
    const double* X;
    int64_t npts;
    int D, Do;
    double* fmean;
    double* fvar;
    int tri;
    double* a2o;
};

template <int NBLK, int RB, int DK, bool BREG, bool TRI = false, int KT = -1>
struct Tile {
    static constexpr int W = (NBLK + RB - 1) / RB;
    static constexpr int NT = 64 * W;
    static constexpr int MP = 16 * NBLK;
    static constexpr int KS = MP / 4;
    static constexpr bool EXACT = (KT >= 0);
    static constexpr int KSE = EXACT ? KS - KT : KS;
    static_assert(!EXACT || (BREG && KT < 4), "the trim applies to register-resident tiles, within the last row block");
    static constexpr int QPW = (4 + W - 1) / W;
    static constexpr int TRI_LDS = TRI ? MP * 16 + 64 : 0;
    static constexpr int LDS_DOUBLES = DK * 64 + MP * 16 + W * 512 + 64 + TRI_LDS;
    static constexpr int NBR = BREG ? (TRI ? KSE + 4 : KSE) : 1;
    static_assert(!(TRI && BREG) || RB == 1, "register-resident triangular operands: one row block per wave");

    __device__ __forceinline__ static int rb_of(int w, int i)
    {
        if constexpr (TRI && BREG && NBLK == 7) {
            return (w == 3) ? 6 : ((w < 3) ? 5 - w : w - 4);
        } else {
            return w * RB + i;
        }
    }
    static constexpr int EPI_LDS_N = BREG ? 0 : (LDS_DOUBLES + 2 * NBLK * 256 <= 20480 ? 2 : (LDS_DOUBLES + NBLK * 256 <= 20480 ? 1 : 0));
    static constexpr bool EPI_LDS = EPI_LDS_N > 0;
    static constexpr int EPI_LDS_DOUBLES = EPI_LDS_N * NBLK * 256;

    double Zreg[RB][DK];
    double czr[RB][4];
    double muA[RB][4];
    double s2A[RB][4];
    double Breg[BREG ? RB : 1][NBR];
    const double* Bp;
    const double* Wp;
    const double* WTp;
    const double* muAg;
    const double* s2Ag;
    int lane_;
    double sigma2;
    int KSr;
    int koff;

    template <bool WITH_EPI = true>
    __device__ __forceinline__ void load_operands(const PackPtrs& pk, int w, int l)
    {
        Bp = pk.Bp;
        Wp = pk.Wp;
        WTp = pk.WTp;
        muAg = pk.muA;
        s2Ag = pk.s2A;
        lane_ = l;
        sigma2 = pk.scal[0];
        KSr = pk.KSr;
        koff = 0;
#pragma unroll
        for (int i = 0; i < RB; ++i) {
// ... 524 lines not shown
#pragma unroll
    for (int qi = 0; qi < TT::QPW; ++qi) {
        const int q = w + qi * TT::W;
        if (q < 4) {
            double fm, fv;
            tile.gather(part, q, l, fm, fv);
            const int d = 4 * q + (l >> 4);
            const int64_t p = p0 + (l & 15);
            if (d < a.Do && p < a.npts) {
                a.fmean[p * a.Do + d] = fm;
                a.fvar[p * a.Do + d] = fv;
            }
        }
    }
}

template <int NBLK, int RB, int DK, bool BREG, int MODE, int NC, bool TRI = false, int KT = -1>
__global__ __launch_bounds__(64 * ((NBLK + RB - 1) / RB)) void pass_kernel(PassArgs a)
{
    static_assert(!TRI || NC == 1, "the two-triangular form runs one column block per workgroup");
    typedef Tile<NBLK, RB, DK, BREG, TRI, KT> TT;
    constexpr int W = TT::W, NT = TT::NT;
    constexpr int NTASK = 4 * NC;
    constexpr int QPW = (NTASK + W - 1) / W;
    constexpr int AUXR = (DK * 64 + NT - 1) / NT;
    constexpr int XS = DK * 64, KTS = TT::MP * 16, PS = W * 512;
    extern __shared__ double lds[];
    double* xq = lds;
    double* Kt = xq + NC * XS;
    double* part = Kt + NC * KTS;
    double* red = part + NC * PS;
    double* At = red + 64 + ((TT::EPI_LDS && NC == 1) ? TT::EPI_LDS_DOUBLES : 0);
    int* flag = reinterpret_cast<int*>(At + TT::MP * 16);

    const int tid = threadIdx.x, l = tid & 63, w = tid >> 6, g = l >> 4, nl = l & 15;
    const int N = a.N, S = a.S, T = a.T, Do = a.Do;
    const int naux = a.D - Do;
    const int gx = blockIdx.x + a.group0;
    const int c0 = gx * 16 * NC;
    const int G16 = (N + 15) >> 4;

    int t_first, nsteps, dir, run = 0, slot = 0;
    const int R = a.recog_len, P = 2 * R;
    if (MODE == MODE_FWD) {
        t_first = 0; nsteps = T - 1; dir = 1;
    } else {
        int k;
        bool dead;
        slot = bwd_segment(blockIdx.y, a.nseg0, gridDim.y, run, k, dead);
        const int o = run * R;
        const int hi = min(P * k - 1 - o, T - 1);
        const int lo = (k > 1) ? (P * (k - 1) - o) : 0;
        t_first = hi; nsteps = dead ? 0 : hi - lo + 1; dir = -1;
        if (nsteps <= 0) {
            if (tid == 0) {
                const int G16p = (a.N + 15) >> 4;
                for (int cq = 0; cq < NC; ++cq)
                    if (gx * NC + cq < G16p) a.part_out[slot * G16p + gx * NC + cq] = (cq == 0) ? 0.0 : 0.0;
            }
            return;
        }
    }

    TT tile;
    tile.load_operands(a.pk, w, l);
    tile.koff = a.ksave ? NBLK * 256 : 0;
    if constexpr (TT::EPI_LDS && NC == 1) {
        double* mul = red + 64;
        for (int i = tid; i < NBLK * 256; i += NT) mul[i] = a.pk.muA[i];
        tile.muAg = mul;
        if constexpr (TT::EPI_LDS_N == 2) {
            double* s2l = mul + NBLK * 256;
            for (int i = tid; i < NBLK * 256; i += NT) s2l[i] = a.pk.s2A[i];
            tile.s2Ag = s2l;
        }
    }

    double vx[QPW], vy[QPW], il[QPW];
    double hcur[QPW];
    double lin[QPW];
    LogProd lp[QPW];
    bool act[QPW], cval[QPW];
    int cc[QPW], bqv[QPW], qv[QPW], cbv[QPW];
#pragma unroll
    for (int qi = 0; qi < QPW; ++qi) {
        const int tk = w + qi * W;
        qv[qi] = tk & 3;
        cbv[qi] = (tk >> 2) < NC ? (tk >> 2) : (NC - 1);
        const int d = 4 * qv[qi] + g;
        const int cg = c0 + cbv[qi] * 16 + nl;
        cc[qi] = min(cg, N - 1);
        cval[qi] = cg < N;
        bqv[qi] = cc[qi] / S;
        act[qi] = (tk < NTASK) && (d < Do);
        const int dc = act[qi] ? d : 0;
        vx[qi] = a.var_x[dc];
        vy[qi] = (MODE == MODE_FWD) ? a.var_y[(a.half && dc >= a.dim_y) ? 0 : dc] : 0.0;
        il[qi] = a.pk.invl[dc];
        lin[qi] = 0.0;
        lp[qi].init();
        hcur[qi] = 0.0;
    }

    const double* auxp[NC][AUXR];
    int auxs[NC][AUXR];
    double auxl[NC][AUXR];
#pragma unroll
    for (int cb = 0; cb < NC; ++cb)
#pragma unroll
        for (int k2 = 0; k2 < AUXR; ++k2) {
            const int i = tid + k2 * NT, ja = i >> 4, n = i & 15;
            auxp[cb][k2] = a.pk.invl; auxs[cb][k2] = 0; auxl[cb][k2] = 0.0;
            if (i < 16 * naux) {
                const int b = min(c0 + cb * 16 + n, N - 1) / S;
                if (ja < a.dim_u) { auxp[cb][k2] = a.u + int64_t(b) * T * a.dim_u + ja; auxs[cb][k2] = a.dim_u; }
                else { auxp[cb][k2] = a.y + int64_t(b) * T * a.dim_y + (ja - a.dim_u); auxs[cb][k2] = a.dim_y; }
                auxl[cb][k2] = a.pk.invl[Do + ja];
            }
        }
    auto aux_load = [&](int cb, int k2, int t) -> double { return auxp[cb][k2][int64_t(t) * auxs[cb][k2]]; };

    for (int i = tid; i < NC * XS; i += NT) xq[i] = 0.0;
    if constexpr (TRI) {
        if (tid < 64) { flag[tid] = 0; flag[tid + 64] = 0; }
    }
    __syncthreads();
    const bool resample0 = (MODE == MODE_BWD) && (((t_first + 1 + run * R) % P) == 0);
    const int tm0 = (MODE == MODE_BWD) ? (t_first % P) : 0;
#pragma unroll
    for (int qi = 0; qi < QPW; ++qi) {
        const int d = 4 * qv[qi] + g;
        const int c = cc[qi];
        if (act[qi]) {
            double v;
            if (MODE == MODE_FWD) {
                if (a.half) v = a.x0[int64_t(bqv[qi]) * a.dim_x + d];
                else v = (d < a.dim_y) ? a.y[(int64_t(bqv[qi]) * T) * a.dim_y + d]
                                       : a.y2_in[int64_t(c) * (a.dim_x - a.dim_y) + (d - a.dim_y)];
                if (cval[qi]) a.x_out[int64_t(c) * a.dim_x + d] = v;
            } else {
                v = resample0 ? a.hid[(int64_t(run) * T + t_first) * N + c] : 0.0;
            }
            hcur[qi] = v;
            xq[cbv[qi] * XS + 64 * qv[qi] + l] = v * il[qi];
        }
    }
    double auxr[NC][AUXR];
#pragma unroll
    for (int cb = 0; cb < NC; ++cb)
#pragma unroll
        for (int k2 = 0; k2 < AUXR; ++k2) {
            const int i = tid + k2 * NT;
            if (i < 16 * naux) xq[cb * XS + 16 * Do + i] = aux_load(cb, k2, t_first) * auxl[cb][k2];
        }

    CBF_STAMP_DECL;
    CBF_STAMP_START();
    for (int step = 0; step < nsteps; ++step) {
        const int t = t_first + dir * step;
        const int tn = t + dir;
        int tmod = tm0 - step; if (tmod < 0) tmod += P;
        const int tmn = (tmod == 0) ? P - 1 : tmod - 1;
        const bool has_next = (step + 1 < nsteps);
        CBF_STAMP_BARRIER(0);

        double eps_t[QPW], ytil[QPW], hidn[QPW];
        bool resample_n = false;
        if (MODE == MODE_BWD) resample_n = has_next && (tmn + 1 + run * R == P);
#pragma unroll
        for (int qi = 0; qi < QPW; ++qi) {
            const int c = cc[qi];
            const int d = 4 * qv[qi] + g;
            ytil[qi] = 0.0; hidn[qi] = 0.0;
            if (MODE == MODE_FWD) {
                eps_t[qi] = a.eps[int64_t(t) * N + c];
                if (act[qi]) {
                    if (d < a.dim_y) ytil[qi] = a.y[(int64_t(bqv[qi]) * T + (t + 1)) * a.dim_y + d];
                    else if (!a.half) ytil[qi] = a.y2_in[(int64_t(t + 1) * N + c) * (a.dim_x - a.dim_y) + (d - a.dim_y)];
                }
            } else {
                eps_t[qi] = a.eps[(int64_t(run) * T + t) * N + c];
                if (resample_n) hidn[qi] = a.hid[(int64_t(run) * T + tn) * N + c];
            }
        }
#pragma unroll
        for (int cb = 0; cb < NC; ++cb)
#pragma unroll
            for (int k2 = 0; k2 < AUXR; ++k2) {
                const int i = tid + k2 * NT;
                auxr[cb][k2] = has_next ? aux_load(cb, k2, tn) : 0.0;
            }

        double* a2o = nullptr;
        if (a.a2s) {
            const int64_t slot = (MODE == MODE_FWD) ? int64_t(t) : (int64_t(run) * T + t);
            a2o = a.a2s + (slot * G16 + int64_t(gx) * NC) * (NBLK * 256 + tile.koff);
        }
        if constexpr (NC == 1) {
            double kr[RB][4];
            tile.phase1(xq, Kt, kr, w, l);
#pragma unroll
            for (int qi = 0; qi < QPW; ++qi) asm volatile("" : "+v"(eps_t[qi]), "+v"(ytil[qi]), "+v"(hidn[qi]));
#pragma unroll
            for (int cb = 0; cb < NC; ++cb)
#pragma unroll
                for (int k2 = 0; k2 < AUXR; ++k2) asm volatile("" : "+v"(auxr[cb][k2]));
            if constexpr (TRI) {
                if (a2o && tile.koff) {
#pragma unroll
                    for (int i = 0; i < RB; ++i) {
                        const int rb = tile.rb_of(w, i);
                        if (rb < NBLK) {
#pragma unroll
                            for (int r = 0; r < 4; ++r) a2o[tile.koff + rb * 256 + r * 64 + l] = kr[i][r];
                        }
                    }
                }
            }
            CBF_STAMP_BARRIER(1);
            if constexpr (TRI) tile.phase2_tri(Kt, At, flag, step + 1, part, w, l, a2o);
            else tile.phase2(Kt, part, kr, w, l, a2o);
        } else {
            tile.template gp_phases<NC>(xq, Kt, part, w, l, a2o, G16 - gx * NC);
        }
        CBF_STAMP_BARRIER(2);

#pragma unroll
        for (int qi = 0; qi < QPW; ++qi) {
            const int tk = w + qi * W;
            if (tk < NTASK) {
                const int q = qv[qi], cb = cbv[qi], c = cc[qi];
                double fm, fv;
                tile.gather(part + cb * PS, q, l, fm, fv);
                const int d = 4 * q + g;
                double outv = 0.0;
                if (act[qi]) {
                    const double fmean = fm + hcur[qi];
                    const double fvar = fv + vx[qi];
                    if (a.fmv && cval[qi]) {
                        const int64_t slot = (MODE == MODE_FWD) ? int64_t(t) : (int64_t(run) * T + t);
                        double* o = a.fmv + ((slot * N + c) * Do + d) * 2;
                        o[0] = fmean; o[1] = fvar;
                    }
                    if (MODE == MODE_FWD) {
                        const double vyt = vy[qi] + (a.k_factor - 1.0) * fvar;
                        const double s = vyt + fvar;
                        const double rs = fast_rcp(s);
                        const double kk = fvar * rs;
                        const double ydiff = ytil[qi] - fmean;
                        const double dm = kk * ydiff;
                        const double mu = fmean + dm;
                        const double sig = kk * vyt;
                        const bool do_cond = (a.condition || (t < R - 1)) && !(a.half && d >= a.dim_y);
                        outv = do_cond ? (mu + eps_t[qi] * (sig * fast_rsqrt(sig)))
                                       : (fmean + eps_t[qi] * (fvar * fast_rsqrt(fvar)));
                        if (do_cond && cval[qi]) {
                            lin[qi] += kk * (ydiff * ydiff * rs - 1.0);
                            lp[qi].mul(vyt * rs);
                        }
                        if (cval[qi]) a.x_out[(int64_t(t + 1) * N + c) * a.dim_x + d] = outv;
                    } else {
                        outv = fmean + eps_t[qi] * (fvar * fast_rsqrt(fvar));
                        const bool write = (run == 0) ? (tmod < R) : (tmod >= R);
                        if (cval[qi]) {
                            if (write) {
                                a.y2_out[(int64_t(t) * N + c) * Do + d] = outv;
                                lp[qi].mul(fvar);
                                lin[qi] += 1.0;
                            }
                            if (a.h_all) a.h_all[((int64_t(run) * T + t) * N + c) * Do + d] = outv;
                        }
                    }
                }
                const double hn = (MODE == MODE_BWD && resample_n) ? hidn[qi] : outv;
                hcur[qi] = act[qi] ? hn : 0.0;
                if (has_next && act[qi]) xq[cb * XS + 64 * q + l] = hn * il[qi];
            }
        }
        if (has_next) {
#pragma unroll
            for (int cb = 0; cb < NC; ++cb)
#pragma unroll
                for (int k2 = 0; k2 < AUXR; ++k2) {
                    const int i = tid + k2 * NT;
                    if (i < 16 * naux) xq[cb * XS + 16 * Do + i] = auxr[cb][k2] * auxl[cb][k2];
                }
        }
    }

    double v = 0.0;
#pragma unroll
    for (int qi = 0; qi < QPW; ++qi) {
        if (act[qi] && cval[qi]) {
            if (MODE == MODE_FWD) v += 0.5 * (lin[qi] - lp[qi].log());
            else v += 0.5 * (lin[qi] * 2.8378770664093453391 + lp[qi].log());
        }
    }
    double tot = block_sum(v, red, tid, NT);
    if constexpr (TRI) {
        if (tid == 0 && flag[CBF_FLAG_TIMEOUT_SLOT] != 0) tot = __builtin_nan("");
    }
    if (tid == 0) {
        const int G16p = (a.N + 15) >> 4;
        for (int cq = 0; cq < NC; ++cq)
            if (gx * NC + cq < G16p) a.part_out[slot * G16p + gx * NC + cq] = (cq == 0) ? tot : 0.0;
    }
#ifdef CBF_REV_STAMPS
#ifndef CBF_STAMP_WAVE_PASS
#define CBF_STAMP_WAVE_PASS (W - 1)
#endif
    if (a.dbg && l == 0 && (w == 0 || w == CBF_STAMP_WAVE_PASS)) {
        double* o = a.dbg + (int64_t(slot) * a.gtotal + gx) * 64 + (w == 0 ? 0 : 32);
        for (int i = 0; i < 7; ++i) { o[i] = double(st_c[i]); o[7 + i] = double(st_w[i]); }
        for (int i = 0; i < 12; ++i) o[14 + i] = double(st_m[i]);
    }
#endif
}

template <int NBLK, int RB, int DK, bool BREG, int MODE, int KT = -1>
__global__ __launch_bounds__(64 * ((NBLK + RB - 1) / RB)) void pass_kernel_skew(PassArgs a)
{
    typedef Tile<NBLK, RB, DK, BREG, false, KT> TT;
    constexpr int W = TT::W, NT = TT::NT;
    constexpr int QPW = TT::QPW;
    constexpr int AUXR = (DK * 64 + NT - 1) / NT;
    constexpr int XS = DK * 64, KTS = TT::MP * 16, PS = W * 512;
    extern __shared__ double lds[];
    double* xq = lds;
    double* Kt = xq + 2 * XS;
    double* part = Kt + 2 * KTS;
    double* red = part + 2 * PS;

    const int tid = threadIdx.x, l = tid & 63, w = tid >> 6, g = l >> 4, nl = l & 15;
    const int N = a.N, S = a.S, T = a.T, Do = a.Do;
    const int naux = a.D - Do;
    const int gx = blockIdx.x + a.group0;
    const int c0 = gx * 32;

    int t_first, nsteps, dir, run = 0, slot = 0;
    const int R = a.recog_len, P = 2 * R;
    if (MODE == MODE_FWD) {
        t_first = 0; nsteps = T - 1; dir = 1;
    } else {
        int k;
        bool dead;
        slot = bwd_segment(blockIdx.y, a.nseg0, gridDim.y, run, k, dead);
        const int o = run * R;
        const int hi = min(P * k - 1 - o, T - 1);
        const int lo = (k > 1) ? (P * (k - 1) - o) : 0;
        t_first = hi; nsteps = dead ? 0 : hi - lo + 1; dir = -1;
        if (nsteps <= 0) {
            if (tid == 0) {
                const int G16p = (a.N + 15) >> 4;
                for (int cq = 0; cq < 2; ++cq)
                    if (gx * 2 + cq < G16p) a.part_out[slot * G16p + gx * 2 + cq] = (cq == 0) ? 0.0 : 0.0;
            }
            return;
        }
    }

    TT tile;
    tile.load_operands(a.pk, w, l);
    tile.koff = a.ksave ? NBLK * 256 : 0;

    double vx[2][QPW], vy[2][QPW], il[2][QPW], hcur[2][QPW], lin[2][QPW];
    LogProd lp[2][QPW];
    bool act[2][QPW], cval[2];
    int cc[2], bqv[2];
#pragma unroll
    for (int c = 0; c < 2; ++c) {
        const int cg = c0 + c * 16 + nl;
        cc[c] = min(cg, N - 1);
        cval[c] = cg < N;
        bqv[c] = cc[c] / S;
        const int wq = (c == 0) ? w : (W - 1 - w);
#pragma unroll
        for (int qi = 0; qi < QPW; ++qi) {
            const int q = wq + qi * W;
            const int d = 4 * q + g;
            act[c][qi] = (q < 4) && (d < Do);
            const int dc = act[c][qi] ? d : 0;
            vx[c][qi] = a.var_x[dc];
            vy[c][qi] = (MODE == MODE_FWD) ? a.var_y[dc] : 0.0;
            il[c][qi] = a.pk.invl[dc];
            lin[c][qi] = 0.0;
            lp[c][qi].init();
            hcur[c][qi] = 0.0;
        }
    }

    const double* auxp[2][AUXR];
    int auxs[2][AUXR];
    double auxl[2][AUXR];
#pragma unroll
    for (int cb = 0; cb < 2; ++cb)
#pragma unroll
        for (int k2 = 0; k2 < AUXR; ++k2) {
            const int i = tid + k2 * NT, ja = i >> 4, n = i & 15;
            auxp[cb][k2] = a.pk.invl; auxs[cb][k2] = 0; auxl[cb][k2] = 0.0;
            if (i < 16 * naux) {
                const int b = min(c0 + cb * 16 + n, N - 1) / S;
                if (ja < a.dim_u) { auxp[cb][k2] = a.u + int64_t(b) * T * a.dim_u + ja; auxs[cb][k2] = a.dim_u; }
                else { auxp[cb][k2] = a.y + int64_t(b) * T * a.dim_y + (ja - a.dim_u); auxs[cb][k2] = a.dim_y; }
                auxl[cb][k2] = a.pk.invl[Do + ja];
            }
        }
    auto aux_load = [&](int cb, int k2, int t) -> double { return auxp[cb][k2][int64_t(t) * auxs[cb][k2]]; };

    for (int i = tid; i < 2 * XS; i += NT) xq[i] = 0.0;
    __syncthreads();
    const bool resample0 = (MODE == MODE_BWD) && (((t_first + 1 + run * R) % P) == 0);
    const int tm0 = (MODE == MODE_BWD) ? (t_first % P) : 0;
#pragma unroll
    for (int c = 0; c < 2; ++c) {
        const int wq = (c == 0) ? w : (W - 1 - w);
#pragma unroll
        for (int qi = 0; qi < QPW; ++qi) {
            const int q = wq + qi * W;
            const int d = 4 * q + g;
            if (act[c][qi]) {
                double v;
                if (MODE == MODE_FWD) {
                    v = (d < a.dim_y) ? a.y[(int64_t(bqv[c]) * T) * a.dim_y + d]
                                      : a.y2_in[int64_t(cc[c]) * (a.dim_x - a.dim_y) + (d - a.dim_y)];
                    if (cval[c]) a.x_out[int64_t(cc[c]) * a.dim_x + d] = v;
                } else {
                    v = resample0 ? a.hid[(int64_t(run) * T + t_first) * N + cc[c]] : 0.0;
                }
                hcur[c][qi] = v;
                xq[c * XS + 64 * q + l] = v * il[c][qi];
            }
        }
#pragma unroll
        for (int k2 = 0; k2 < AUXR; ++k2) {
            const int i = tid + k2 * NT;
            if (i < 16 * naux) xq[c * XS + 16 * Do + i] = aux_load(c, k2, t_first) * auxl[c][k2];
        }
    }
    __syncthreads();

    double kregA[RB][4], kregB[RB][4];

    auto phase3 = [&](auto cidx, int s) {
        constexpr int c = decltype(cidx)::value;
        const int t = t_first + dir * s;
        const int tn = t + dir;
        int tmod = tm0 - s; if (tmod < 0) tmod += P;
        const int tmn = (tmod == 0) ? P - 1 : tmod - 1;
        const bool has_next = (s + 1 < nsteps);
        const int wq = (c == 0) ? w : (W - 1 - w);
        const int cch = cc[c];
        bool resample_n = false;
        if (MODE == MODE_BWD) resample_n = has_next && (tmn + 1 + run * R == P);
        double eps_t, hidn = 0.0;
        if (MODE == MODE_FWD) eps_t = a.eps[int64_t(t) * N + cch];
        else {
            eps_t = a.eps[(int64_t(run) * T + t) * N + cch];
            if (resample_n) hidn = a.hid[(int64_t(run) * T + tn) * N + cch];
        }
        double auxn[AUXR];
#pragma unroll
        for (int k2 = 0; k2 < AUXR; ++k2) {
            const int i = tid + k2 * NT;
            auxn[k2] = has_next ? aux_load(c, k2, tn) : 0.0;
        }
#pragma unroll
        for (int qi = 0; qi < QPW; ++qi) {
            const int q = wq + qi * W;
            if (q < 4) {
                const int d = 4 * q + g;
                double ytil = 0.0;
                if (MODE == MODE_FWD && act[c][qi])
                    ytil = (d < a.dim_y) ? a.y[(int64_t(bqv[c]) * T + (t + 1)) * a.dim_y + d]
                                         : a.y2_in[(int64_t(t + 1) * N + cch) * (a.dim_x - a.dim_y) + (d - a.dim_y)];
                double fm, fv;
                tile.gather(part + c * PS, q, l, fm, fv);
                double outv = 0.0;
                if (act[c][qi]) {
                    const double fmean = fm + hcur[c][qi];
                    const double fvar = fv + vx[c][qi];
                    if (a.fmv && cval[c]) {
                        const int64_t slot = (MODE == MODE_FWD) ? int64_t(t) : (int64_t(run) * T + t);
                        double* o = a.fmv + ((slot * N + cch) * Do + d) * 2;
                        o[0] = fmean; o[1] = fvar;
                    }
                    if (MODE == MODE_FWD) {
                        const double vyt = vy[c][qi] + (a.k_factor - 1.0) * fvar;
                        const double sm = vyt + fvar;
                        const double rs = fast_rcp(sm);
                        const double kk = fvar * rs;
                        const double ydiff = ytil - fmean;
                        const double mu = fmean + kk * ydiff;
                        const double sig = kk * vyt;
                        const bool do_cond = a.condition || (t < R - 1);
                        outv = do_cond ? (mu + eps_t * (sig * fast_rsqrt(sig))) : (fmean + eps_t * (fvar * fast_rsqrt(fvar)));
                        if (do_cond && cval[c]) {
                            lin[c][qi] += kk * (ydiff * ydiff * rs - 1.0);
                            lp[c][qi].mul(vyt * rs);
                        }
                        if (cval[c]) a.x_out[(int64_t(t + 1) * N + cch) * a.dim_x + d] = outv;
                    } else {
                        outv = fmean + eps_t * (fvar * fast_rsqrt(fvar));
                        const bool write = (run == 0) ? (tmod < R) : (tmod >= R);
                        if (cval[c]) {
                            if (write) {
                                a.y2_out[(int64_t(t) * N + cch) * Do + d] = outv;
                                lp[c][qi].mul(fvar);
                                lin[c][qi] += 1.0;
                            }
                            if (a.h_all) a.h_all[((int64_t(run) * T + t) * N + cch) * Do + d] = outv;
                        }
                    }
                }
                const double hn = (MODE == MODE_BWD && resample_n) ? hidn : outv;
                hcur[c][qi] = act[c][qi] ? hn : 0.0;
                if (has_next && act[c][qi]) xq[c * XS + 64 * q + l] = hn * il[c][qi];
            }
        }
        if (has_next) {
#pragma unroll
            for (int k2 = 0; k2 < AUXR; ++k2) {
                const int i = tid + k2 * NT;
                if (i < 16 * naux) xq[c * XS + 16 * Do + i] = auxn[k2] * auxl[c][k2];
            }
        }
    };
    using I0 = std::integral_constant<int, 0>;
    using I1 = std::integral_constant<int, 1>;

    const int G16 = (N + 15) >> 4;
    auto a2slot = [&](int s, int c) -> double* {
        if (!a.a2s || 2 * gx + c >= G16) return nullptr;
        const int t = t_first + dir * s;
        const int64_t slot = (MODE == MODE_FWD) ? int64_t(t) : (int64_t(run) * T + t);
        return a.a2s + (slot * G16 + 2 * gx + c) * (NBLK * 256 + tile.koff);
    };
    tile.phase1(xq, Kt, kregA, w, l);
    __syncthreads();
    const bool hi = (w >= 4);
    for (int s = 0; s < nsteps; ++s) {
        if (hi) {
            if (s > 0) phase3(I1{}, s - 1);
            tile.phase2(Kt, part, kregA, w, l, a2slot(s, 0));
        } else {
            tile.phase2(Kt, part, kregA, w, l, a2slot(s, 0));
            if (s > 0) phase3(I1{}, s - 1);
        }
        __syncthreads();
        if (hi) {
            tile.phase1(xq + XS, Kt + KTS, kregB, w, l);
            phase3(I0{}, s);
        } else {
            phase3(I0{}, s);
            tile.phase1(xq + XS, Kt + KTS, kregB, w, l);
        }
        __syncthreads();
        if (hi) {
            tile.phase2(Kt + KTS, part + PS, kregB, w, l, a2slot(s, 1));
            if (s + 1 < nsteps) tile.phase1(xq, Kt, kregA, w, l);
        } else {
            if (s + 1 < nsteps) tile.phase1(xq, Kt, kregA, w, l);
            tile.phase2(Kt + KTS, part + PS, kregB, w, l, a2slot(s, 1));
        }
        __syncthreads();
    }
    phase3(I1{}, nsteps - 1);

    double v = 0.0;
#pragma unroll
    for (int c = 0; c < 2; ++c)
#pragma unroll
        for (int qi = 0; qi < QPW; ++qi) {
            if (act[c][qi] && cval[c]) {
                if (MODE == MODE_FWD) v += 0.5 * (lin[c][qi] - lp[c][qi].log());
                else v += 0.5 * (lin[c][qi] * 2.8378770664093453391 + lp[c][qi].log());
            }
        }
    const double tot = block_sum(v, red, tid, NT);
    if (tid == 0) {
        const int G16p = (a.N + 15) >> 4;
        for (int cq = 0; cq < 2; ++cq)
            if (gx * 2 + cq < G16p) a.part_out[slot * G16p + gx * 2 + cq] = (cq == 0) ? tot : 0.0;
    }
}

}
```

cbf-ssm_amd/csrc/cbfssm_tail.hip:

```cpp
#include <hip/hip_runtime.h>
#include <stdint.h>
#include <string.h>

#include "../../include/cbfssm_hip.h"

namespace cbfssm {

int fail(int rc, const char* fmt, ...);

struct GpTail {
    const double* slab;
    const double* gB_dense;
    int64_t gB_ld;
    const double* Kinv;
    const double* Kmm;
    const double* Zs;
    double* T;
    double* G2;
    double* dv;
    const double* scal;
    const double* zmean;
    const double* zvar;
    const double* ls;
    const double* var;
// ... 219 lines not shown
        p.g_z[idx] = gzt / p.ls[p.shared_ls ? 0 : j];
    }
    __syncthreads();
    for (int j = wv; j < D; j += NT / 64) {
        double s = 0.0;
        for (int i = l; i < M; i += 64) s += p.g_z[i * D + j] * p.Zs[i * D + j];
        for (int o = 32; o > 0; o >>= 1) s += __shfl_xor(s, o);
        if (l == 0) {
            const double sx = nd ? 0.0 : small[32 + j];
            if (p.shared_ls) glsj[j] = -(s + sx / p.ls[0]);
            else p.g_ls[j] = -(s + sx / p.ls[j]) * sigmoid(p.ls_unc[j]);
        }
    }
    if (p.shared_ls) {
        __syncthreads();
        if (tid == 0) {
            double s = 0.0;
            for (int j = 0; j < D; ++j) s += glsj[j];
            p.g_ls[0] = s * sigmoid(p.ls_unc[0]);
        }
    }
    if (tid == 0) {
        const double var = p.var[0];
        const double s96 = nd ? 0.0 : small[96], s97 = nd ? 0.0 : small[97];
        p.g_var[0] = (tot / var + s96 + s97 / var) * sigmoid(p.var_unc[0]);
    }
    for (int idx = tid; idx < M * Do; idx += NT) {
        const int i = idx / Do, d = idx - i * Do;
        const double gm0 = nd ? 0.0 : c_image(gMu, 1, i, d), gs0 = nd ? 0.0 : c_image(gS2, 1, i, d);
        p.g_mu[idx] = gm0 + p.klw * KM[idx];
        const double gs2 = gs0 + p.klw * 0.5 * ((p.Kkl ? p.Kkl : p.Kinv)[int64_t(i) * M + i] - 1.0 / p.zvar[idx]);
        p.g_s2[idx] = gs2 * sigmoid(p.zvar_unc[idx]);
    }
    if (blockIdx.x == 0 && tid < a.dim_x) {
        double gvx = small[tid];
        if (a.ngp > 1) {
            const GpTail& pb = a.gp[1];
            const double* small_b = pb.slab + 2 * pb.NBLK * 256 + (pb.stash ? 0 : pb.NBLK * pb.NBLK * 256) + pb.NBLK * pb.JB * 256;
            if (tid < pb.Do) gvx += small_b[tid];
        }
        a.g_vx[tid] = gvx * sigmoid(a.vx_unc[tid]);
        if (tid < a.n_vy) {
            double gvy = small[16 + tid];
            if (tid < a.dim_y) gvy += a.tail[3 + tid];
            a.g_vy[tid] = gvy * sigmoid(a.vy_unc[tid]);
        }
    }
}

struct ConstrainArgs {
    const double* p;
    double* c;
    int64_t off[13];
    int unc[12];
};

__global__ __launch_bounds__(256) void constrain_kernel(ConstrainArgs a)
{
    const int64_t i = int64_t(blockIdx.x) * 256 + threadIdx.x;
    if (i >= a.off[12]) return;
    int seg = 0;
#pragma unroll
    for (int s = 1; s < 12; ++s) seg += (i >= a.off[s]);
    const double x = a.p[i];
    a.c[i] = a.unc[seg] ? (fmax(x, 0.0) + log1p(exp(-fabs(x))) + 1e-10) : x;
}

__global__ __launch_bounds__(256) void data_tail_kernel(const double* ll_part, int64_t nblk, int dim_y, const double* var_y,
                                                        const double* out8, double cL, double bts, double* tail)
{
    __shared__ double red[4];
    const int tid = threadIdx.x, d = blockIdx.x;
    double s = 0.0;
    for (int64_t k = tid; k < nblk; k += 256) s += ll_part[k * dim_y + d];
    const double tot = block_sum_t(s, red, tid, 256);
    if (tid == 0) {
        const double vy = var_y[d];
        const double sq = (-2.0 * tot - bts * (1.8378770664093454836 + log(vy))) * vy;
        tail[3 + d] = -cL * 0.5 * (sq / (vy * vy) - bts / vy);
    }
    if (d == 0 && tid < 3) tail[tid] = out8[tid];
}

__global__ void adam_tick_kernel(double* t) { t[0] += 1.0; }

__global__ __launch_bounds__(256) void adam_kernel(int64_t n, double* p, const double* g, double* m, double* v, const double* t,
                                                   double lr, double b1, double b2, double eps)
{
    const int64_t i = int64_t(blockIdx.x) * 256 + threadIdx.x;
    if (i >= n) return;
    const double tt = t[0];
    const double lr_t = lr * sqrt(1.0 - pow(b2, tt)) / (1.0 - pow(b1, tt));
    const double gi = g[i];
    const double mi = b1 * m[i] + (1.0 - b1) * gi;
    const double vi = b2 * v[i] + (1.0 - b2) * gi * gi;
    m[i] = mi;
    v[i] = vi;
    p[i] -= lr_t * mi / (sqrt(vi) + eps);
}

}

namespace cbfssm {

static int one_gp_tail(const cbfssm_pack_layout* L, const double* pack, const double* pack_kl, int shared_ls, const double* slab,
                       const double* gB_dense, int64_t gB_ld, int g_mode, double klw, int dim_y, const double* pflat,
                       const double* cflat, double* work, double* gflat, void* stream, const char* what)
{
    TailArgs a;
    memset(&a, 0, sizeof(a));
    GpTail& p = a.gp[0];
    const int M = L->M, D = L->D, Do = L->Do;
    p.slab = slab;
    p.gB_dense = gB_dense; p.gB_ld = gB_ld;
    p.Kinv = pack + L->Kinv; p.Kmm = pack + L->Kmm; p.Zs = pack + L->Zs;
    double* w = work;
    p.T = w; w += int64_t(M) * (M > 48 ? M : 48);
    p.G2 = w; w += int64_t(M) * M;
    p.T2 = w; w += int64_t(M) * M;
    p.dv = w;
    p.scal = pack + L->scal;
    p.Kkl = pack_kl ? pack_kl + L->Kinv : nullptr;
    p.shared_ls = shared_ls ? 1 : 0;
    p.klw = klw; p.nodata = slab ? 0 : 1;
    const int64_t o1 = int64_t(M) * D, o2 = o1 + int64_t(M) * Do, o3 = o2 + int64_t(M) * Do, o4 = o3 + 1,
                  o5 = o4 + (shared_ls ? 1 : D), o6 = o5 + Do;
    p.zmean = cflat + o1; p.zvar = cflat + o2; p.var = cflat + o3; p.ls = cflat + o4;
    p.zvar_unc = pflat + o2; p.var_unc = pflat + o3; p.ls_unc = pflat + o4;
    p.g_z = gflat; p.g_mu = gflat + o1; p.g_s2 = gflat + o2; p.g_var = gflat + o3; p.g_ls = gflat + o4;
    p.M = M; p.D = D; p.Do = Do; p.NBLK = L->NBLK; p.JB = L->JB; p.stash = L->rev_stash; p.gmode = g_mode;
    a.ngp = 1;
    if (dim_y > 0) {
        a.tail = slab + L->rev_slab;
        a.vx_unc = pflat + o5; a.vy_unc = pflat + o6;
        a.g_vx = gflat + o5; a.g_vy = gflat + o6;
        a.dim_x = Do; a.dim_y = dim_y; a.n_vy = dim_y;
    }
    const unsigned nb = unsigned((M + 15) / 16);
    hipStream_t st = (hipStream_t)stream;
    hipLaunchKernelGGL(tail_gemm<0>, dim3(nb, nb, 1), dim3(16, 16), 0, st, a);
    if (pack_kl) hipLaunchKernelGGL(tail_gemm<3>, dim3(nb, nb, 1), dim3(16, 16), 0, st, a);
    hipLaunchKernelGGL(tail_gemm<1>, dim3(nb, nb, 1), dim3(16, 16), 0, st, a);
    hipLaunchKernelGGL(tail_gemm<2>, dim3(3, nb, 1), dim3(16, 16), 0, st, a);
    hipLaunchKernelGGL(tail_finish, dim3(1), dim3(256), 0, st, a);
    hipError_t e = hipGetLastError();
    return e == hipSuccess ? 0 : fail(-int(e) - 1000, "%s", what);
}

}

using namespace cbfssm;

extern "C" {

int cbfssm_param_layout_init(int M, int dim_x, int dim_u, int dim_y, cbfssm_param_layout* out)
{
    if (!out) return fail(-1, "null layout");
    if (M < 1 || dim_x < 1 || dim_u < 0 || dim_y < 1 || dim_y > dim_x) return fail(-1, "bad dimensions");
    const int D = dim_x + dim_u;
    const int Do[2] = {dim_x, dim_x - dim_y};
    int64_t o = 0;
    int k = 0;
    for (int g = 0; g < 2; ++g) {
        out->off[k++] = o; o += int64_t(M) * D;
        out->off[k++] = o; o += int64_t(M) * Do[g];
        out->off[k++] = o; o += int64_t(M) * Do[g];
// ... 62 lines not shown
    const double* slab = red;
    double* w = work;
    for (int g = 0; g < 2; ++g) {
        GpTail& p = a.gp[g];
        const int M = L[g]->M;
        p.slab = slab; slab += L[g]->rev_slab;
        p.gB_dense = gBd[g]; p.gB_ld = gB_ld;
        p.Kinv = pack[g] + L[g]->Kinv; p.Kmm = pack[g] + L[g]->Kmm; p.Zs = pack[g] + L[g]->Zs;
        p.T = w; w += int64_t(M) * (M > 48 ? M : 48);
        p.G2 = w; w += int64_t(M) * M;
        p.dv = w; w += (int64_t(M) + 63) / 64 * 64;
        p.scal = pack[g] + L[g]->scal;
        const int64_t* off = pl->off + 5 * g;
        p.zmean = cflat + off[1]; p.zvar = cflat + off[2]; p.var = cflat + off[3]; p.ls = cflat + off[4];
        p.zvar_unc = pflat + off[2]; p.var_unc = pflat + off[3]; p.ls_unc = pflat + off[4];
        p.g_z = gflat + off[0]; p.g_mu = gflat + off[1]; p.g_s2 = gflat + off[2]; p.g_var = gflat + off[3];
        p.g_ls = gflat + off[4];
        p.M = M; p.D = L[g]->D; p.Do = L[g]->Do; p.NBLK = L[g]->NBLK; p.JB = L[g]->JB; p.stash = L[g]->rev_stash;
        p.gmode = g_mode;
        p.Kkl = nullptr; p.T2 = nullptr; p.shared_ls = 0;
        p.klw = 1.0; p.nodata = 0;
    }
    a.ngp = 2; a.n_vy = pl->dim_x;
    a.tail = slab;
    a.vx_unc = pflat + pl->off[10]; a.vy_unc = pflat + pl->off[11];
    a.g_vx = gflat + pl->off[10]; a.g_vy = gflat + pl->off[11];
    a.dim_x = pl->dim_x; a.dim_y = pl->dim_y;
    const unsigned nb = unsigned((pl->M + 15) / 16);
    hipStream_t st = (hipStream_t)stream;
    hipLaunchKernelGGL(tail_gemm<0>, dim3(nb, nb, 2), dim3(16, 16), 0, st, a);
    hipLaunchKernelGGL(tail_gemm<1>, dim3(nb, nb, 2), dim3(16, 16), 0, st, a);
    hipLaunchKernelGGL(tail_gemm<2>, dim3(3, nb, 2), dim3(16, 16), 0, st, a);
    hipLaunchKernelGGL(tail_finish, dim3(2), dim3(256), 0, st, a);
    hipError_t e = hipGetLastError();
    return e == hipSuccess ? 0 : fail(-int(e) - 1000, "train tail launch failed");
}

int64_t cbfssm_train_tail_half_work_elems(const cbfssm_pack_layout* L)
{
    if (!L) return -1;
    return int64_t(L->M) * (L->M > 48 ? L->M : 48) + 2 * int64_t(L->M) * L->M + (int64_t(L->M) + 63) / 64 * 64;
}

int cbfssm_train_tail_half_f64(const cbfssm_pack_layout* L, const double* pack, const double* pack_kl, int shared_ls,
                               const double* red, const double* gB_dense, int64_t gB_ld, int g_mode, int dim_y, const double* pflat,
                               const double* cflat, double* work, double* gflat, void* stream)
{
    if (g_mode < 0 || g_mode > 2) return fail(-1, "g_mode must be 0, 1 or 2");
    if (!L || !pack || !red || !pflat || !cflat || !work || !gflat) return fail(-1, "null pointer");
    if (L->rev_slab <= 0) return fail(-3, "no adjoint slab for M=%d", L->M);
    if (L->M > 320 || L->D > 32) return fail(-3, "tail kernel limits: M <= 320, D <= 32");
    if ((L->rev_stash != 0) != (gB_dense != nullptr)) return fail(-1, "the dense K^-1 adjoint is required exactly in stash mode");
    if (dim_y < 1 || dim_y > L->Do) return fail(-1, "bad dim_y");
    return one_gp_tail(L, pack, pack_kl, shared_ls, red, gB_dense, gB_ld, g_mode, 1.0, dim_y, pflat, cflat, work, gflat, stream,
                       "train tail (forward-only variant) launch failed");
}

int cbfssm_gp_tail_f64(const cbfssm_pack_layout* L, const double* pack, const double* red_slab, const double* gB_dense,
                       int64_t gB_ld, double kl_weight, const double* pflat, const double* cflat, double* work, double* gflat,
                       void* stream)
{
    if (!L || !pack || !pflat || !cflat || !work || !gflat) return fail(-1, "null pointer");
    if (L->rev_slab <= 0) return fail(-3, "no adjoint slab for M=%d", L->M);
    if (L->M < 1 || L->M > 320 || L->D < 1 || L->D > 32 || L->Do < 1 || L->Do > CBFSSM_MAX_DOUT)
        return fail(-3, "tail kernel limits: M <= 320, D <= 32, Do <= %d", CBFSSM_MAX_DOUT);
    if (red_slab && (L->rev_stash != 0) != (gB_dense != nullptr))
        return fail(-1, "the dense K^-1 adjoint is required exactly in stash mode");
    if (!red_slab && gB_dense) return fail(-1, "a K^-1 adjoint without a slab");
    return one_gp_tail(L, pack, nullptr, 0, red_slab, gB_dense, gB_ld, 0, kl_weight, 0, pflat, cflat, work, gflat, stream,
                       "gp tail launch failed");
}

int cbfssm_data_tail_f64(const cbfssm_problem* p, const double* var_y, const double* ll_part, const double* out8, double cL,
                         double* tail, void* stream)
{
    if (!p || !var_y || !ll_part || !out8 || !tail) return fail(-1, "null pointer");
    const int64_t nblk = (int64_t(p->B) * p->T * p->dim_x + 255) / 256;
    hipLaunchKernelGGL(data_tail_kernel, dim3(unsigned(p->dim_y > 0 ? p->dim_y : 1)), dim3(256), 0, (hipStream_t)stream, ll_part, nblk, p->dim_y, var_y, out8, cL,
                       double(p->B) * p->T * p->S, tail);
    hipError_t e = hipGetLastError();
    return e == hipSuccess ? 0 : fail(-int(e) - 1000, "data tail launch failed");
}

int cbfssm_adam_step_f64(int64_t n, double* pflat, const double* gflat, double* m, double* v, double* t_dev, double lr,
                         double beta1, double beta2, double eps, void* stream)
{
    if (n < 1 || !pflat || !gflat || !m || !v || !t_dev) return fail(-1, "null pointer");
    hipStream_t st = (hipStream_t)stream;
    hipLaunchKernelGGL(adam_tick_kernel, dim3(1), dim3(1), 0, st, t_dev);
    hipLaunchKernelGGL(adam_kernel, dim3(unsigned((n + 255) / 256)), dim3(256), 0, st, n, pflat, gflat, m, v,
                       (const double*)t_dev, lr, beta1, beta2, eps);
    hipError_t e = hipGetLastError();
    return e == hipSuccess ? 0 : fail(-int(e) - 1000, "adam launch failed");
}

}
```

include/cbfssm_hip.h:

```cpp
#ifndef CBFSSM_HIP_H
#define CBFSSM_HIP_H

#include <stddef.h>
#include <stdint.h>

#ifdef __cplusplus
extern "C" {
#endif

#define CBFSSM_MAX_DOUT 16
#define CBFSSM_MAX_DIN 64
#define CBFSSM_MAX_M 320

enum {
    CBFSSM_SCAL_SIGMA2 = 0,
    CBFSSM_SCAL_LOGDET = 1,
    CBFSSM_SCAL_KLZ = 2,
    CBFSSM_SCAL_INFO = 3,
    CBFSSM_SCAL_COND = 4,
    CBFSSM_SCAL_JITTER = 5,
    CBFSSM_SCAL_COUNT = 16
};

enum {
// ... 69 lines not shown
int64_t cbfssm_gp_predict_bwd_workgroups(const cbfssm_pack_layout* layout, int64_t npts);
int64_t cbfssm_gp_predict_bwd_work_elems(const cbfssm_pack_layout* layout, int64_t npts);
int cbfssm_gp_predict_bwd_f64(const cbfssm_pack_layout* layout, const double* pack, const double* X, int64_t npts,
                              const double* gmean, const double* gvar, double* gX, double* gpart, double* work,
                              double* gB_image, void* stream);
int cbfssm_gp_tail_f64(const cbfssm_pack_layout* layout, const double* pack, const double* red_slab, const double* gB_dense,
                       int64_t gB_ld, double kl_weight, const double* pflat, const double* cflat, double* work, double* gflat,
                       void* stream);

int64_t cbfssm_gp_rollout_partials(const cbfssm_pack_layout* layout, int64_t N);
int cbfssm_gp_rollout_f64(const cbfssm_pack_layout* layout, const double* pack, const double* h0, const double* a,
                          const double* eps, const double* var_add, int64_t N, int64_t T, int reverse, double* traj,
                          double* vsave, double* ent_part, void* stream);
int64_t cbfssm_gp_rollout_bwd_workgroups(const cbfssm_pack_layout* layout, int64_t N);
int64_t cbfssm_gp_rollout_bwd_work_elems(const cbfssm_pack_layout* layout, int64_t N, int64_t T);
int cbfssm_gp_rollout_bwd_f64(const cbfssm_pack_layout* layout, const double* pack, const double* h0, const double* a,
                              const double* eps, const double* traj, const double* vsave, const double* gtraj,
                              const double* g_ent, int64_t N, int64_t T, int reverse, double* gh0, double* ga,
                              double* gpart, double* work, double* gB_image, void* stream);

int64_t cbfssm_gp_filter_partials(const cbfssm_pack_layout* layout, int64_t N);
int cbfssm_gp_filter_f64(const cbfssm_pack_layout* layout, const double* pack, const double* h0, const double* a,
                         const double* ytilde, const double* cond, const double* eps, const double* var_x,
                         const double* var_y, double k_factor, int64_t N, int64_t T, int reverse, double* traj,
                         double* msave, double* vsave, double* kl_part, void* stream);
int64_t cbfssm_gp_filter_bwd_workgroups(const cbfssm_pack_layout* layout, int64_t N);
int64_t cbfssm_gp_filter_bwd_work_elems(const cbfssm_pack_layout* layout, int64_t N, int64_t T);
int cbfssm_gp_filter_bwd_f64(const cbfssm_pack_layout* layout, const double* pack, const double* h0, const double* a,
                             const double* ytilde, const double* cond, const double* eps, const double* var_y,
                             double k_factor, const double* traj, const double* msave, const double* vsave,
                             const double* gtraj, const double* g_kl, int64_t N, int64_t T, int reverse, double* gh0,
                             double* ga, double* gytilde, double* gpart, double* work, double* gB_image,
                             void* stream);

typedef struct cbfssm_rigid_body {
    double mass_inv;
    double inertia_inv[3];
    double gravity[3];
    double dt;
} cbfssm_rigid_body;
int64_t cbfssm_rigid_filter_partials(int64_t N);
int cbfssm_rigid_filter_f64(const cbfssm_rigid_body* body, const double* x0, const double* u, const double* y,
                            const double* eps, const double* var_x, const double* var_y, int64_t N, int64_t S,
                            double* traj, double* kl_part, void* stream);
int cbfssm_rigid_filter_bwd_f64(const cbfssm_rigid_body* body, const double* x0, const double* u, const double* y,
                                const double* eps, const double* var_x, const double* var_y, const double* traj,
                                const double* gtraj, const double* g_kl, int64_t N, int64_t S, double* gx0, double* gu,
                                double* gy, double* gpart, void* stream);

int64_t cbfssm_backward_pass_partials(const cbfssm_problem* p);
int cbfssm_backward_pass_f64(const cbfssm_problem* p, const cbfssm_pack_layout* layout_b, const double* pack_b,
                             const double* var_x, const double* u, const double* y, const double* hid_b,
                             const double* eps_b, double* y2, double* h_all, double* fmv_b, double* a2s_b,
                             double* ent_part, void* stream);

int64_t cbfssm_forward_pass_partials(const cbfssm_problem* p);

int64_t cbfssm_saved_a2_elems(const cbfssm_problem* p, const cbfssm_pack_layout* layout, int backward);
int cbfssm_forward_pass_f64(const cbfssm_problem* p, const cbfssm_pack_layout* layout_f, const double* pack_f,
                            const double* var_x, const double* var_y, const double* u, const double* y,
                            const double* y2, const double* eps_f, double* x, double* fmv_f, double* a2s_f,
                            double* kl_part, void* stream);

int cbfssm_half_forward_pass_f64(const cbfssm_problem* p, const cbfssm_pack_layout* layout_f, const double* pack_f,
                                 const double* var_x, const double* var_y, const double* u, const double* y,
                                 const double* x0, const double* eps_f, double* x, double* fmv_f, double* a2s_f,
                                 double* kl_part, void* stream);
int cbfssm_half_forward_pass_bwd_f64(const cbfssm_problem* p, const cbfssm_pack_layout* layout_f, const double* pack_f,
                                     const double* var_x, const double* var_y, const double* u, const double* y,
                                     const double* eps_f, const double* x, const double* fmv_f, const double* a2s_f, double cL,
                                     double* gx0, double* gpart, int t_hi, int t_lo, double* gx_carry, double* stash_a,
                                     double* stash_k, int64_t stash_ld, void* stream);

int64_t cbfssm_loglik_partials(const cbfssm_problem* p);
int cbfssm_loglik_moments_f64(const cbfssm_problem* p, const double* var_y, const double* y, const double* x,
                              double* ll_part, double* pred_mean, double* pred_var, double* int_mean,
                              double* int_var, void* stream);

int cbfssm_elbo_combine_f64(const cbfssm_problem* p, double lambda0, double lambda1,
                            const double* ll_part, int64_t n_ll, const double* kl_part, int64_t n_kl,
                            const double* ent_part, int64_t n_ent, const double* scal_f, const double* scal_b,
                            double* out, void* stream);

int64_t cbfssm_rev_workgroups(const cbfssm_problem* p, int backward_runs);

int cbfssm_bwd_schedule(const cbfssm_problem* p, int cap, int* run, int* t_begin, int* nsteps);

int cbfssm_forward_pass_bwd_f64(const cbfssm_problem* p, const cbfssm_pack_layout* layout_f, const double* pack_f,
                                const double* var_x, const double* var_y, const double* u, const double* y,
                                const double* y2, const double* eps_f, const double* x, const double* fmv_f,
                                const double* a2s_f, double cL, double* gy2, double* gpart, void* stream);

int cbfssm_backward_pass_bwd_f64(const cbfssm_problem* p, const cbfssm_pack_layout* layout_b, const double* pack_b,
                                 const double* var_x, const double* u, const double* y, const double* hid_b,
                                 const double* eps_b, const double* h_all, const double* fmv_b, const double* a2s_b,
                                 const double* gy2, double cE, double* gpart, void* stream);

int cbfssm_bwd_segments(const cbfssm_problem* p);
int cbfssm_forward_pass_bwd_ex_f64(const cbfssm_problem* p, const cbfssm_pack_layout* layout_f, const double* pack_f,
                                   const double* var_x, const double* var_y, const double* u, const double* y,
                                   const double* y2, const double* eps_f, const double* x, const double* fmv_f,
                                   const double* a2s_f, double cL, double* gy2, double* gpart, int t_hi, int t_lo,
                                   double* gx_carry, double* stash_a, double* stash_k, int64_t stash_ld, void* stream);
int cbfssm_backward_pass_bwd_ex_f64(const cbfssm_problem* p, const cbfssm_pack_layout* layout_b, const double* pack_b,
                                    const double* var_x, const double* u, const double* y, const double* hid_b,
                                    const double* eps_b, const double* h_all, const double* fmv_b, const double* a2s_b,
                                    const double* gy2, double cE, double* gpart, int seg0, int seg1, int nchunk,
                                    double* stash_a, double* stash_k, int64_t stash_ld, void* stream);

int64_t cbfssm_input_adjoint_fwd_elems(const cbfssm_problem* p);
int64_t cbfssm_input_adjoint_bwd_elems(const cbfssm_problem* p);
int64_t cbfssm_input_adjoint_obs_elems(const cbfssm_problem* p);
int cbfssm_forward_pass_bwd_in_f64(const cbfssm_problem* p, const cbfssm_pack_layout* layout_f, const double* pack_f,
                                   const double* var_x, const double* var_y, const double* u, const double* y,
                                   const double* y2, const double* eps_f, const double* x, const double* fmv_f,
                                   const double* a2s_f, double cL, double* gy2, double* gpart, int t_hi, int t_lo,
                                   double* gx_carry, double* stash_a, double* stash_k, int64_t stash_ld, double* gin_f,
                                   double* gyo, void* stream);
int cbfssm_backward_pass_bwd_in_f64(const cbfssm_problem* p, const cbfssm_pack_layout* layout_b, const double* pack_b,
                                    const double* var_x, const double* u, const double* y, const double* hid_b,
                                    const double* eps_b, const double* h_all, const double* fmv_b, const double* a2s_b,
                                    const double* gy2, double cE, double* gpart, int seg0, int seg1, int nchunk,
                                    double* stash_a, double* stash_k, int64_t stash_ld, double* gin_b, void* stream);
int cbfssm_input_grads_f64(const cbfssm_problem* p, const cbfssm_pack_layout* layout_f, const double* pack_f,
                           const cbfssm_pack_layout* layout_b, const double* pack_b, const double* var_y, const double* y,
                           const double* x, const double* gin_f, const double* gin_b, const double* gyo, double cL,
                           double* grad_u, double* grad_y, void* stream);

#define CBFSSM_REDUCE_SPLIT 32
int cbfssm_reduce_partials_f64(double* gpart, int64_t slab, int64_t nwg, double* out, void* stream);

int64_t cbfssm_stash_contract_work_elems(const cbfssm_pack_layout* layout, int64_t nslots);
int cbfssm_stash_contract_f64(const cbfssm_pack_layout* layout, const double* stash_a, const double* stash_k, int64_t nslots,
                              double* work, double* ginv_image, void* stream);

int64_t cbfssm_pack_f32_elems(const cbfssm_pack_layout* layout);
int cbfssm_gp_pack_f32(const cbfssm_pack_layout* layout, const double* pack, float* pack32, void* stream);
int cbfssm_gp_pack_bf16(const cbfssm_pack_layout* layout, const double* pack, float* pack32, void* stream);
int cbfssm_gp_predict_f32(const cbfssm_pack_layout* layout, const float* pack32, const double* X, int64_t npts,
                          double* fmean, double* fvar, void* stream);
int cbfssm_backward_pass_f32(const cbfssm_problem* p, const cbfssm_pack_layout* layout_b, const float* pack32_b,
                             const double* var_x, const double* u, const double* y, const double* hid_b,
                             const double* eps_b, double* y2, double* h_all, double* fmv_b, float* a2s_b, double* ent_part,
                             void* stream);
int cbfssm_forward_pass_f32(const cbfssm_problem* p, const cbfssm_pack_layout* layout_f, const float* pack32_f,
                            const double* var_x, const double* var_y, const double* u, const double* y,
                            const double* y2, const double* eps_f, double* x, double* fmv_f, float* a2s_f, double* kl_part,
                            void* stream);
int64_t cbfssm_saved_a2_f32_elems(const cbfssm_problem* p, const cbfssm_pack_layout* layout, int backward_runs);
int cbfssm_half_forward_pass_f32(const cbfssm_problem* p, const cbfssm_pack_layout* layout_f, const float* pack32_f,
                                 const double* var_x, const double* var_y, const double* u, const double* y,
                                 const double* x0, const double* eps_f, double* x, double* fmv_f, float* a2s_f,
                                 double* kl_part, void* stream);
int cbfssm_half_forward_pass_bwd_f32(const cbfssm_problem* p, const cbfssm_pack_layout* layout_f, const float* pack32_f,
                                     const double* var_x, const double* var_y, const double* u, const double* y,
                                     const double* eps_f, const double* x, const double* fmv_f, const float* a2s_f, double cL,
                                     double* gx0, double* gpart, void* stream);
int64_t cbfssm_rev32_slab_elems(const cbfssm_pack_layout* layout);
int cbfssm_forward_pass_bwd_f32(const cbfssm_problem* p, const cbfssm_pack_layout* layout_f, const float* pack32_f,
                                const double* var_x, const double* var_y, const double* u, const double* y,
                                const double* y2, const double* eps_f, const double* x, const double* fmv_f, const float* a2s_f,
                                double cL, double* gy2, double* gpart, void* stream);
int cbfssm_backward_pass_bwd_f32(const cbfssm_problem* p, const cbfssm_pack_layout* layout_b, const float* pack32_b,
                                 const double* var_x, const double* u, const double* y, const double* hid_b,
                                 const double* eps_b, const double* h_all, const double* fmv_b, const float* a2s_b,
                                 const double* gy2, double cE, double* gpart, void* stream);

typedef struct cbfssm_param_layout {
    int64_t off[12];
    int64_t total;
    int32_t M, D, dim_x, dim_y;
} cbfssm_param_layout;

int cbfssm_param_layout_init(int M, int dim_x, int dim_u, int dim_y, cbfssm_param_layout* out);

int cbfssm_constrain_f64(const cbfssm_param_layout* pl, const double* pflat, double* cflat, void* stream);

int64_t cbfssm_train_tail_work_elems(const cbfssm_pack_layout* layout_f, const cbfssm_pack_layout* layout_b);

int cbfssm_train_tail_f64(const cbfssm_param_layout* pl, const cbfssm_pack_layout* layout_f, const double* pack_f,
                          const cbfssm_pack_layout* layout_b, const double* pack_b, const double* red,
                          const double* gB_dense_f, const double* gB_dense_b, int64_t gB_ld, const double* pflat,
                          const double* cflat, double* work, double* gflat, void* stream);
int cbfssm_train_tail_g_f64(const cbfssm_param_layout* pl, const cbfssm_pack_layout* layout_f, const double* pack_f,
                            const cbfssm_pack_layout* layout_b, const double* pack_b, const double* red,
                            const double* gB_dense_f, const double* gB_dense_b, int64_t gB_ld, int g_mode, const double* pflat,
                            const double* cflat, double* work, double* gflat, void* stream);

int64_t cbfssm_train_tail_half_work_elems(const cbfssm_pack_layout* layout);
int cbfssm_train_tail_half_f64(const cbfssm_pack_layout* layout, const double* pack, const double* pack_kl, int shared_ls,
                               const double* red, const double* gB_dense, int64_t gB_ld, int g_mode, int dim_y,
                               const double* pflat, const double* cflat, double* work, double* gflat, void* stream);

int64_t cbfssm_gru_recog_param_elems(int dim_u, int dim_y, int dim_x);
int64_t cbfssm_gru_recog_act_elems(int B, int recog_len);
int cbfssm_gru_recog_f64(int B, int T, int dim_u, int dim_y, int dim_x, int recog_len, const double* u, const double* y,
                         const double* params, double* x0, double* act, void* stream);
int cbfssm_gru_recog_bwd_f64(int B, int T, int dim_u, int dim_y, int dim_x, int recog_len, const double* u, const double* y,
                             const double* params, const double* act, const double* gx0, double* gpart, void* stream);

int64_t cbfssm_conv_recog_param_elems(int dim_u, int dim_y, int dim_x, int recog_len);
int cbfssm_conv_recog_f32(int B, int T, int dim_u, int dim_y, int dim_x, int recog_len, const double* u, const double* y,
                          const double* params, double* x0, void* stream);
int cbfssm_conv_recog_bwd_f32(int B, int T, int dim_u, int dim_y, int dim_x, int recog_len, const double* u, const double* y,
                              const double* params, const double* gx0, double* gpart, void* stream);

int cbfssm_gru_recog_bwd_in_f64(int B, int T, int dim_u, int dim_y, int dim_x, int recog_len, const double* u, const double* y,
                                const double* params, const double* act, const double* gx0, double* gpart, double* gwin,
                                void* stream);
int cbfssm_conv_recog_bwd_in_f32(int B, int T, int dim_u, int dim_y, int dim_x, int recog_len, const double* u, const double* y,
                                 const double* params, const double* gx0, double* gpart, double* gwin, void* stream);
int cbfssm_half_forward_pass_bwd_in_f64(const cbfssm_problem* p, const cbfssm_pack_layout* layout_f, const double* pack_f,
                                        const double* var_x, const double* var_y, const double* u, const double* y,
// ... 23 lines not shown
```

Before: 98.38 steps/s (one step = one 256-sequence mini-batch per GPU).

## Fuse log-likelihood squared residuals into forward pass and defer moments off critical path

The forward pass kernel now accumulates per-group squared residuals between observations and sampled states, so the ELBO combine and data tail read compact partials instead of waiting on the separate loglik moments kernel. The moments kernel, which is still needed for predictions, is deferred until after the adjoint passes and runs on a side stream joined by an event, and the forward-partials reduction is issued earlier. The HIP graph path also captures graphs that alias the noise buffers directly once the same pointers reappear, avoiding per-step noise copies. This adds extra registers and a shuffle reduction to the forward kernel and more complex graph and stream bookkeeping.

Result: no change. 99.25 steps/s (one step = one 256-sequence mini-batch per GPU) (median of 6 runs) (+0.9%).

```diff
diff --git a/cbf-ssm_amd/cbfssm/hip/lib.py b/cbf-ssm_amd/cbfssm/hip/lib.py
--- a/cbf-ssm_amd/cbfssm/hip/lib.py
+++ b/cbf-ssm_amd/cbfssm/hip/lib.py
@@ -31,6 +31,7 @@
     'cbfssm_rigid_filter_partials', 'cbfssm_rigid_filter_f64', 'cbfssm_rigid_filter_bwd_f64',
     'cbfssm_gru_recog_bwd_in_f64', 'cbfssm_conv_recog_bwd_in_f32', 'cbfssm_half_forward_pass_bwd_in_f64',
     'cbfssm_half_input_grads_f64',
+    'cbfssm_forward_pass_sq_f64', 'cbfssm_elbo_combine_sq_f64', 'cbfssm_data_tail_sq_f64',
 )
 
 
@@ -129,6 +130,9 @@
     lib.cbfssm_half_forward_pass_f64.argtypes = [C.POINTER(Problem), C.POINTER(PackLayout)] + [vp] * 12
     lib.cbfssm_half_forward_pass_bwd_f64.argtypes = ([C.POINTER(Problem), C.POINTER(PackLayout)] + [vp] * 9 + [dbl, vp, vp, ip, ip, vp, vp, vp, i64, vp])
     lib.cbfssm_reduce_partials_f64.argtypes = [vp, i64, i64, vp, vp]
+    lib.cbfssm_forward_pass_sq_f64.argtypes = [C.POINTER(Problem), C.POINTER(PackLayout)] + [vp] * 13
+    lib.cbfssm_elbo_combine_sq_f64.argtypes = [C.POINTER(Problem), dbl, dbl, vp, vp, vp, i64, vp, i64, vp, vp, vp, vp]
+    lib.cbfssm_data_tail_sq_f64.argtypes = [C.POINTER(Problem), vp, vp, vp, dbl, vp, vp]
     lib.cbfssm_cholesky_f64.argtypes = [ip, vp, dbl, vp, vp, vp, vp]
     lib.cbfssm_rbf_k_f64.argtypes = [ip, ip, ip, vp, vp, vp, vp, vp, vp]
     lib.cbfssm_gp_predict_fullq_work_elems.restype = i64
diff --git a/cbf-ssm_amd/cbfssm/hip/ops.py b/cbf-ssm_amd/cbfssm/hip/ops.py
--- a/cbf-ssm_amd/cbfssm/hip/ops.py
+++ b/cbf-ssm_amd/cbfssm/hip/ops.py
@@ -273,6 +273,7 @@
         self.ent_part = torch.zeros(self.n_ent, **f)
         self.kl_part = torch.zeros(self.n_kl, **f)
         self.ll_part = torch.zeros(int(lib.cbfssm_loglik_partials(C.byref(p))), **f)
+        self.sq_part = torch.zeros(self.n_kl * max(p.dim_y, 1), **f)
         self.pred_mean = torch.zeros(p.B, T, p.dim_y, **f)
         self.pred_var = torch.zeros(p.B, T, p.dim_y, **f)
         self.int_mean = torch.zeros(p.B, T, p.dim_x, **f)
@@ -293,6 +294,7 @@
         self.var_x, self.var_y, self.u, self.y, self.x0, self.eps_f, self.hid_b, self.eps_b = \
             var_x, var_y, u, y, x0, eps_f, hid_b, eps_b
         self.cL, self.cE, self.f32, self.bf16 = cL, cE, f32, bf16
+        self.ll_in_pass = False
         self.in_bufs = None
 
     def cast_f32(self):
@@ -323,7 +325,11 @@
 
     def forward_pass(self, q, st):
         lib = _l.load()
-        a = self._fwd_args(q, self.ws.y2) + (_ptr(self.ws.kl_part), st)
+        a = self._fwd_args(q, self.ws.y2) + (_ptr(self.ws.kl_part),)
+        if self.ll_in_pass:
+            _l.check(lib.cbfssm_forward_pass_sq_f64(*a, _ptr(self.ws.sq_part), st), 'cbfssm_forward_pass_sq_f64')
+            return
+        a = a + (st,)
         self._check(lib.cbfssm_forward_pass_f32(*a) if self.f32 else lib.cbfssm_forward_pass_f64(*a), 'forward_pass')
 
     def forward_pass_bwd(self, q, st, chunk=None):
@@ -397,11 +403,29 @@
                                                        _ptr(gx0), _ptr(gwin), int(recog_len), self.cL, _ptr(grad_u),
                                                        _ptr(grad_y), st), 'cbfssm_half_input_grads_f64')
 
+    def moments(self, st):
+        lib, ws = _l.load(), self.ws
+        _l.check(lib.cbfssm_loglik_moments_f64(C.byref(self.prob), _ptr(self.var_y), _ptr(self.y), _ptr(ws.x), _ptr(ws.ll_part),
+                                               _ptr(ws.pred_mean), _ptr(ws.pred_var), _ptr(ws.int_mean),
+                                               _ptr(ws.int_var), st), 'cbfssm_loglik_moments_f64')
+
+    def combine_sq(self, lf0, lf1, st):
+        lib, ws = _l.load(), self.ws
+        _l.check(lib.cbfssm_elbo_combine_sq_f64(C.byref(self.prob), float(lf0), float(lf1), _ptr(ws.sq_part),
+                                                _ptr(self.var_y), _ptr(ws.kl_part), ws.kl_part.numel(), _ptr(ws.ent_part),
+                                                ws.ent_part.numel(), _ptr(self.pack_f.scal), _ptr(self.pack_b.scal),
+                                                _ptr(ws.out), st), 'cbfssm_elbo_combine_sq_f64')
+
+    def tail(self, lf0, lf1, st):
+        if self.ll_in_pass:
+            self.combine_sq(lf0, lf1, st)
+            self.moments(st)
+        else:
+            self.elbo_tail(lf0, lf1, st)
+
     def elbo_tail(self, lf0, lf1, st, kl_pack=None):
         lib, ws, pb = _l.load(), self.ws, C.byref(self.prob)
-        _l.check(lib.cbfssm_loglik_moments_f64(pb, _ptr(self.var_y), _ptr(self.y), _ptr(ws.x), _ptr(ws.ll_part),
-                                               _ptr(ws.pred_mean), _ptr(ws.pred_var), _ptr(ws.int_mean),
-                                               _ptr(ws.int_var), st), 'cbfssm_loglik_moments_f64')
+        self.moments(st)
         b = self.pack_b is not None
         _l.check(lib.cbfssm_elbo_combine_f64(pb, float(lf0), float(lf1), _ptr(ws.ll_part), ws.ll_part.numel(),
                                              _ptr(ws.kl_part), ws.kl_part.numel(), _ptr(ws.ent_part) if b else None,
@@ -410,7 +434,7 @@
                  'cbfssm_elbo_combine_f64')
 
 
-def elbo_forward(lp, loss_factors):
+def elbo_forward(lp, loss_factors, defer_tail=False):
     prob, st = lp.prob, _stream()
     N = prob.B * prob.S
     assert lp.u.shape == (prob.B, prob.T, prob.dim_u) and lp.y.shape == (prob.B, prob.T, prob.dim_y)
@@ -419,7 +443,8 @@
     lp.cast_f32()
     lp.backward_pass(prob, st)
     lp.forward_pass(prob, st)
-    lp.elbo_tail(loss_factors[0], loss_factors[1], st)
+    if not defer_tail:
+        lp.tail(loss_factors[0], loss_factors[1], st)
     return lp.ws
 
 
diff --git a/cbf-ssm_amd/cbfssm/hip/train.py b/cbf-ssm_amd/cbfssm/hip/train.py
--- a/cbf-ssm_amd/cbfssm/hip/train.py
+++ b/cbf-ssm_amd/cbfssm/hip/train.py
@@ -303,8 +303,10 @@
         lp = self._loops(prob, ws, c, u, y, noise)
         if input_grads:
             lp.in_bufs = self._input_buffers(prob, ws)
-        self._elbo_forward(lp)
-        if self.stash and not self.f32:
+        lp.ll_in_pass = not self.f32 and prob.dim_y >= 1 and not os.environ.get('CBFSSM_NO_LL_IN_PASS')
+        stash = self.stash and not self.f32
+        self._elbo_forward(lp, defer_tail=lp.ll_in_pass and not stash)
+        if stash:
             gB_f, gB_b = self._adjoint_stash(lp, self.red)
         else:
             gB_f, gB_b = self._adjoint(lp, self.red)
@@ -312,9 +314,18 @@
             lp.input_grads(ws.grad_u, ws.grad_y, _stream())
         sf, sb = self.slab_f, self.slab_b
         tail = self.red[sf + sb:sf + sb + self.ntail]
-        _l.check(_l.load().cbfssm_data_tail_f64(C.byref(prob), _ptr(c['var_y']), _ptr(ws.ll_part), _ptr(ws.out), lp.cL,
-                                          _ptr(tail), _stream()), 'cbfssm_data_tail_f64')
-        return dict(ws=ws, p=p, c=c, pflat=pflat, gB_f=gB_f, gB_b=gB_b, cL=lp.cL, cE=lp.cE, input_grads=bool(input_grads))
+        if lp.ll_in_pass:
+            _l.check(_l.load().cbfssm_data_tail_sq_f64(C.byref(prob), _ptr(c['var_y']), _ptr(ws.sq_part), _ptr(ws.out), lp.cL,
+                                                       _ptr(tail), _stream()), 'cbfssm_data_tail_sq_f64')
+        else:
+            _l.check(_l.load().cbfssm_data_tail_f64(C.byref(prob), _ptr(c['var_y']), _ptr(ws.ll_part), _ptr(ws.out), lp.cL,
+                                                    _ptr(tail), _stream()), 'cbfssm_data_tail_f64')
+        join = getattr(lp, 'join', None)
+        if join is not None and self.dist is not None:
+            torch.cuda.current_stream().wait_event(join)
+            join = None
+        return dict(ws=ws, p=p, c=c, pflat=pflat, gB_f=gB_f, gB_b=gB_b, cL=lp.cL, cE=lp.cE, input_grads=bool(input_grads),
+                    join=join)
 
     def _grads_finish(self, s):
         lib = _l.load()
@@ -342,6 +353,8 @@
             grads = self._grads_tensor_library(p, c, red, tail, gB_f, gB_b)
         if s.get('input_grads'):
             grads['u'], grads['y'] = ws.grad_u, ws.grad_y
+        if s.get('join') is not None:
+            torch.cuda.current_stream().wait_event(s['join'])
         return loss, grads, terms
 
     def _grads_tensor_library(self, p, c, red, tail, gB_f, gB_b):
@@ -401,11 +414,11 @@
         return (self._sub_problem(prob, 0, main), self._sub_problem(prob, main, rest), s0, s1,
                 C.c_void_p(s0.cuda_stream), C.c_void_p(s1.cuda_stream))
 
-    def _elbo_forward(self, lp):
+    def _elbo_forward(self, lp, defer_tail=False):
         lf = self.config['loss_factors']
         split = self._split(lp.prob, adjoint=False)
         if split is None:
-            ops.elbo_forward(lp, lf)
+            ops.elbo_forward(lp, lf, defer_tail)
             return
         p_main, p_rest, s0, s1, st0, st1 = self._two_streams(lp.prob, split)
         lp.cast_f32()
@@ -419,15 +432,21 @@
         e1.record(s1)
         s0.wait_event(e1)
         lp.forward_pass(p_main, st0)
-        lp.elbo_tail(lf[0], lf[1], st0)
+        if not defer_tail:
+            lp.tail(lf[0], lf[1], st0)
 
     def _adjoint(self, lp, red):
         ws, st = lp.ws, _stream()
         sf, sb = self.slab_f, self.slab_b
         split = self._split(lp.prob, adjoint=False)
+        early_f = False
+        lf = self.config['loss_factors']
+        lp.join = None
         if split is None:
             lp.forward_pass_bwd(lp.prob, st)
             lp.backward_pass_bwd(lp.prob, st)
+            if lp.ll_in_pass:
+                lp.tail(lf[0], lf[1], st)
         else:
             p_main, p_rest, s0, s1, st0, st1 = self._two_streams(lp.prob, split)
             lp.forward_pass_bwd(p_main, st0)
@@ -439,12 +458,27 @@
             e3 = torch.cuda.Event()
             e3.record(s1)
             lp.backward_pass_bwd(p_rest, st0)
+            if not self.repack32:
+                ops.reduce_partials(ws.gpart_f, sf, ws.n_f, red[:sf], st0)
+                early_f = True
+            if lp.ll_in_pass:
+                lp.combine_sq(lf[0], lf[1], st0)
             s0.wait_event(e3)
         if not self.repack32:
             assert not self.f32 or (self.slab32_f, self.slab32_b) == (sf, sb)
-            ops.reduce_partials(ws.gpart_f, sf, ws.n_f, red[:sf], st)
+            if not early_f:
+                ops.reduce_partials(ws.gpart_f, sf, ws.n_f, red[:sf], st)
             ops.reduce_partials(ws.gpart_b, sb, ws.n_b, red[sf:sf + sb], st)
+            if split is not None and lp.ll_in_pass:
+                e4 = torch.cuda.Event()
+                e4.record(s0)
+                s1.wait_event(e4)
+                lp.moments(st1)
+                lp.join = torch.cuda.Event()
+                lp.join.record(s1)
             return None, None
+        if split is not None and lp.ll_in_pass:
+            lp.moments(st)
         if self._tmp32 is None:
             self._tmp32 = torch.zeros(self.slab32_f + self.slab32_b, dtype=torch.float64, device=self.device)
         tf, tb = self._tmp32[:self.slab32_f], self._tmp32[self.slab32_f:]
@@ -677,6 +711,7 @@
             graph = config.get('hip_graph', os.environ.get('CBFSSM_HIP_GRAPH', '1') != '0')
         self.use_graph = bool(graph) and not self.engine.stash
         self._graphs = {}
+        self.alias_noise = not self.engine.f32 and not os.environ.get('CBFSSM_GRAPH_NOISE_COPY')
         self.last_ws = None
 
     def step(self, u, y, noise, condition=True, weight=1.0, local=False):
@@ -688,56 +723,75 @@
         self.last_ws = self.engine.last_ws
         return loss
 
+    def _capture(self, u, y, noise, condition, weight, alias):
+        dev = self.engine.device
+        g = {'u': u.clone(), 'y': y.clone(), 'noise': noise, 'alias': alias}
+        cur = torch.cuda.current_stream(dev)
+        side = torch.cuda.Stream(device=dev)
+        side.wait_stream(cur)
+        with torch.cuda.stream(side):
+            self.engine.loss_and_grads(self.params, g['u'], g['y'], g['noise'], condition, local=True)
+        cur.wait_stream(side)
+        eng = self.engine
+        front = None
+        t_before = self.opt._t
+        mode = 'global' if eng.dist is None else 'thread_local'
+        try:
+            if eng.dist is not None:
+                torch.cuda.synchronize(dev)
+                front = torch.cuda.CUDAGraph()
+                with torch.cuda.graph(front, capture_error_mode=mode):
+                    state = eng._grads_local(self.params, g['u'], g['y'], g['noise'], condition)
+            graph = torch.cuda.CUDAGraph()
+            with torch.cuda.graph(graph, capture_error_mode=mode):
+                if front is None:
+                    state = eng._grads_local(self.params, g['u'], g['y'], g['noise'], condition)
+                loss, grads, terms = eng._grads_finish(state)
+                if getattr(grads, 'flat', None) is not None:
+                    self.opt.step(grads)
+                else:
+                    self.opt.step_device(grads)
+                self.opt._t -= 1
+        except RuntimeError as e:
+            if eng.dist is None:
+                raise
+            import warnings
+            warnings.warn('HIP graph capture failed on this rank (%s): continuing with eager launches' % e)
+            torch.cuda.synchronize(dev)
+            self.opt._t = t_before
+            self.use_graph = False
+            self._eager_loss = self.step(u, y, noise, condition, weight=weight)
+            return None
+        g.update(graph=graph, front=front, state=state, loss=loss, terms=terms, ws=state['ws'])
+        return g
+
     def _graph_step(self, u, y, noise, condition, weight=1.0):
         dev = self.engine.device
         u, y = _f64(u, dev), _f64(y, dev)
         key = (tuple(u.shape), tuple(y.shape), bool(condition), self.engine.gp_forms())
-        g = self._graphs.get(key)
         names = ('hid_b', 'eps_b', 'eps_f')
+        nz = {k: _f64(noise[k], dev) for k in names}
+        fam = self._graphs.setdefault(key, {'copy': None, 'alias': {}, 'seen': []})
+        ptrs = tuple(nz[k].data_ptr() for k in names)
+        g = fam['alias'].get(ptrs)
         if g is None:
-            g = {'u': u.clone(), 'y': y.clone(), 'noise': {k: _f64(noise[k], dev).clone() for k in names}}
-            cur = torch.cuda.current_stream(dev)
-            side = torch.cuda.Stream(device=dev)
-            side.wait_stream(cur)
-            with torch.cuda.stream(side):
-                self.engine.loss_and_grads(self.params, g['u'], g['y'], g['noise'], condition, local=True)
-            cur.wait_stream(side)
-            eng = self.engine
-            front = None
-            t_before = self.opt._t
-            mode = 'global' if eng.dist is None else 'thread_local'
-            try:
-                if eng.dist is not None:
-                    torch.cuda.synchronize(dev)
-                    front = torch.cuda.CUDAGraph()
-                    with torch.cuda.graph(front, capture_error_mode=mode):
-                        state = eng._grads_local(self.params, g['u'], g['y'], g['noise'], condition)
-                graph = torch.cuda.CUDAGraph()
-                with torch.cuda.graph(graph, capture_error_mode=mode):
-                    if front is None:
-                        state = eng._grads_local(self.params, g['u'], g['y'], g['noise'], condition)
-                    loss, grads, terms = eng._grads_finish(state)
-                    if getattr(grads, 'flat', None) is not None:
-                        self.opt.step(grads)
-                    else:
-                        self.opt.step_device(grads)
-                    self.opt._t -= 1
-            except RuntimeError as e:
-                if eng.dist is None:
-                    raise
-                import warnings
-                warnings.warn('HIP graph capture failed on this rank (%s): continuing with eager launches' % e)
-                torch.cuda.synchronize(dev)
-                self.opt._t = t_before
-                self.use_graph = False
-                return self.step(u, y, noise, condition, weight=weight)
-            g.update(graph=graph, front=front, state=state, loss=loss, terms=terms, ws=state['ws'])
-            self._graphs[key] = g
-        else:
-            g['u'].copy_(u)
-            g['y'].copy_(y)
+            back = any(q == ptrs for q, _ in fam['seen'])
+            if back and len(fam['alias']) < 2 and self.alias_noise:
+                g = fam['alias'][ptrs] = self._capture(u, y, nz, condition, weight, alias=True)
+                fam['seen'] = [e for e in fam['seen'] if e[0] != ptrs]
+            else:
+                if fam['copy'] is None:
+                    fam['copy'] = self._capture(u, y, {k: v.clone() for k, v in nz.items()}, condition, weight, alias=False)
+                g = fam['copy']
+                if not back and len(fam['alias']) < 2 and self.alias_noise:
+                    fam['seen'] = fam['seen'][-1:] + [(ptrs, nz)]
+        if g is None:
+            return self._eager_loss
+        g['u'].copy_(u)
+        g['y'].copy_(y)
+        if not g['alias']:
             for k in names:
-                g['noise'][k].copy_(_f64(noise[k], dev))
+                g['noise'][k].copy_(nz[k])
         if g['front'] is not None:
             g['front'].replay()
             self.engine._grads_collective(g['state'], weight)
diff --git a/cbf-ssm_amd/csrc/cbfssm_api.hip b/cbf-ssm_amd/csrc/cbfssm_api.hip
--- a/cbf-ssm_amd/csrc/cbfssm_api.hip
+++ b/cbf-ssm_amd/csrc/cbfssm_api.hip
@@ -583,6 +583,7 @@
 }
 
 struct CombineArgs {
+    const double* sq; int64_t n_sq; const double* var_y; int dim_y; double bts;
     const double* ll; int64_t n_ll;
     const double* kl; int64_t n_kl;
     const double* ent; int64_t n_ent;
@@ -598,9 +599,13 @@
     const int tid = threadIdx.x;
     double s0 = 0.0, s1 = 0.0, s2 = 0.0;
     for (int64_t i = tid; i < a.n_ll; i += 1024) s0 += a.ll[i];
+    for (int64_t i = tid; i < a.n_sq; i += 1024) s0 += -0.5 * a.sq[i] / a.var_y[i % a.dim_y];
     for (int64_t i = tid; i < a.n_kl; i += 1024) s1 += a.kl[i];
     for (int64_t i = tid; i < a.n_ent; i += 1024) s2 += a.ent[i];
-    const double loglik = block_sum(s0, red, tid, 1024);
+    double loglik = block_sum(s0, red, tid, 1024);
+    if (tid == 0 && a.n_sq > 0) {
+        for (int d = 0; d < a.dim_y; ++d) loglik += -0.5 * a.bts * (1.8378770664093454836 + log(a.var_y[d]));
+    }
     const double kl_x = block_sum(s1, red, tid, 1024);
     const double entropy = block_sum(s2, red, tid, 1024);
     if (tid == 0) {
@@ -1170,7 +1175,7 @@
 static int forward_pass_impl(const cbfssm_problem* p, const cbfssm_pack_layout* L, const double* pack_f,
                              const double* var_x, const double* var_y, const double* u, const double* y,
                              const double* y2, const double* x0, const double* eps_f, double* x, double* fmv_f,
-                             double* a2s_f, double* kl_part, void* stream)
+                             double* a2s_f, double* kl_part, void* stream, double* sq_part = nullptr)
 {
     int rc = check_problem(p, L, p ? p->dim_x : 0);
     if (rc) return rc;
@@ -1185,6 +1190,7 @@
     a.recog_len = p->recog_len; a.condition = p->condition; a.k_factor = p->k_factor;
     a.var_x = var_x; a.var_y = var_y; a.u = u; a.y = y; a.eps = eps_f; a.y2_in = y2; a.x_out = x;
     a.part_out = kl_part;
+    a.sq_out = sq_part;
     a.dbg = g_dbg;
     a.half = p->half; a.x0 = x0;
     a.fmv = fmv_f;
@@ -1211,6 +1217,16 @@
     return forward_pass_impl(p, L, pack_f, var_x, var_y, u, y, y2, nullptr, eps_f, x, fmv_f, a2s_f, kl_part, stream);
 }
 
+int cbfssm_forward_pass_sq_f64(const cbfssm_problem* p, const cbfssm_pack_layout* L, const double* pack_f,
+                               const double* var_x, const double* var_y, const double* u, const double* y,
+                               const double* y2, const double* eps_f, double* x, double* fmv_f, double* a2s_f,
+                               double* kl_part, double* sq_part, void* stream)
+{
+    if (p && p->half) return fail(-1, "problem->half is set: no squared-residual partials for the forward-only variants");
+    if (!sq_part) return fail(-1, "null pointer");
+    return forward_pass_impl(p, L, pack_f, var_x, var_y, u, y, y2, nullptr, eps_f, x, fmv_f, a2s_f, kl_part, stream, sq_part);
+}
+
 int cbfssm_half_forward_pass_f64(const cbfssm_problem* p, const cbfssm_pack_layout* L, const double* pack_f,
                                  const double* var_x, const double* var_y, const double* u, const double* y,
                                  const double* x0, const double* eps_f, double* x, double* fmv_f, double* a2s_f,
@@ -1248,12 +1264,30 @@
 {
     if (!p || !scal_f || !out) return fail(-1, "null pointer");
     CombineArgs a;
+    a.sq = nullptr; a.n_sq = 0; a.var_y = nullptr; a.dim_y = 1; a.bts = 0.0;
     a.ll = ll_part; a.n_ll = ll_part ? n_ll : 0; a.kl = kl_part; a.n_kl = kl_part ? n_kl : 0;
     a.ent = ent_part; a.n_ent = ent_part ? n_ent : 0;
     a.scal_f = scal_f; a.scal_b = scal_b; a.lambda0 = lambda0; a.lambda1 = lambda1; a.inv_s = 1.0 / p->S;
     a.out = out;
     hipLaunchKernelGGL(combine_kernel, dim3(1), dim3(1024), 0, (hipStream_t)stream, a);
     return check_launch("elbo_combine");
+}
+
+int cbfssm_elbo_combine_sq_f64(const cbfssm_problem* p, double lambda0, double lambda1, const double* sq_part,
+                               const double* var_y, const double* kl_part, int64_t n_kl, const double* ent_part,
+                               int64_t n_ent, const double* scal_f, const double* scal_b, double* out, void* stream)
+{
+    if (!p || !scal_f || !out || !sq_part || !var_y) return fail(-1, "null pointer");
+    if (p->dim_y < 1) return fail(-1, "bad dim_y");
+    CombineArgs a;
+    a.sq = sq_part; a.n_sq = cbfssm_forward_pass_partials(p) * p->dim_y; a.var_y = var_y; a.dim_y = p->dim_y;
+    a.bts = double(p->B) * p->T * p->S;
+    a.ll = nullptr; a.n_ll = 0; a.kl = kl_part; a.n_kl = kl_part ? n_kl : 0;
+    a.ent = ent_part; a.n_ent = ent_part ? n_ent : 0;
+    a.scal_f = scal_f; a.scal_b = scal_b; a.lambda0 = lambda0; a.lambda1 = lambda1; a.inv_s = 1.0 / p->S;
+    a.out = out;
+    hipLaunchKernelGGL(combine_kernel, dim3(1), dim3(1024), 0, (hipStream_t)stream, a);
+    return check_launch("elbo_combine_sq");
 }
 
 constexpr int SCHED_UNITS = 256;
diff --git a/cbf-ssm_amd/csrc/cbfssm_kernels.hpp b/cbf-ssm_amd/csrc/cbfssm_kernels.hpp
--- a/cbf-ssm_amd/csrc/cbfssm_kernels.hpp
+++ b/cbf-ssm_amd/csrc/cbfssm_kernels.hpp
@@ -303,6 +303,7 @@
     double* fmv;
     int tri;
     int ksave;
+    double* sq_out;
 };
 
 __device__ __forceinline__ int bwd_segment(int y, int n0, int ny, int& run, int& k, bool& dead)
@@ -993,6 +994,8 @@
     LogProd lp[QPW];
     bool act[QPW], cval[QPW];
     int cc[QPW], bqv[QPW], qv[QPW], cbv[QPW];
+    double sq[QPW];
+    bool sqon[QPW];
 #pragma unroll
     for (int qi = 0; qi < QPW; ++qi) {
         const int tk = w + qi * W;
@@ -1011,6 +1014,8 @@
         lin[qi] = 0.0;
         lp[qi].init();
         hcur[qi] = 0.0;
+        sq[qi] = 0.0;
+        sqon[qi] = (MODE == MODE_FWD) && a.sq_out && act[qi] && cval[qi] && (d < a.dim_y);
     }
 
     const double* auxp[NC][AUXR];
@@ -1170,6 +1175,7 @@
                             lp[qi].mul(vyt * rs);
                         }
                         if (cval[qi]) a.x_out[(int64_t(t + 1) * N + c) * a.dim_x + d] = outv;
+                        if (sqon[qi]) { const double r = ytil[qi] - outv; sq[qi] = fma(r, r, sq[qi]); }
                     } else {
                         outv = fmean + eps_t[qi] * (fvar * fast_rsqrt(fvar));
                         const bool write = (run == 0) ? (tmod < R) : (tmod >= R);
@@ -1215,6 +1221,16 @@
         const int G16p = (a.N + 15) >> 4;
         for (int cq = 0; cq < NC; ++cq)
             if (gx * NC + cq < G16p) a.part_out[slot * G16p + gx * NC + cq] = (cq == 0) ? tot : 0.0;
+    }
+    if (MODE == MODE_FWD && a.sq_out) {
+#pragma unroll
+        for (int qi = 0; qi < QPW; ++qi) {
+            double v2 = sq[qi];
+#pragma unroll
+            for (int o = 8; o > 0; o >>= 1) v2 += __shfl_xor(v2, o);
+            const int tk = w + qi * W, d = 4 * qv[qi] + g, grp = gx * NC + cbv[qi];
+            if (tk < NTASK && nl == 0 && d < a.dim_y && d < Do && grp < G16) a.sq_out[int64_t(grp) * a.dim_y + d] = v2;
+        }
     }
 #ifdef CBF_REV_STAMPS
 #ifndef CBF_STAMP_WAVE_PASS
@@ -1275,6 +1291,8 @@
     tile.koff = a.ksave ? NBLK * 256 : 0;
 
     double vx[2][QPW], vy[2][QPW], il[2][QPW], hcur[2][QPW], lin[2][QPW];
+    double sq[2][QPW];
+    bool sqon[2][QPW];
     LogProd lp[2][QPW];
     bool act[2][QPW], cval[2];
     int cc[2], bqv[2];
@@ -1297,6 +1315,8 @@
             lin[c][qi] = 0.0;
             lp[c][qi].init();
             hcur[c][qi] = 0.0;
+            sq[c][qi] = 0.0;
+            sqon[c][qi] = (MODE == MODE_FWD) && a.sq_out && act[c][qi] && cval[c] && (d < a.dim_y);
         }
     }
 
@@ -1410,6 +1430,7 @@
                             lp[c][qi].mul(vyt * rs);
                         }
                         if (cval[c]) a.x_out[(int64_t(t + 1) * N + cch) * a.dim_x + d] = outv;
+                        if (sqon[c][qi]) { const double r = ytil - outv; sq[c][qi] = fma(r, r, sq[c][qi]); }
                     } else {
                         outv = fmean + eps_t * (fvar * fast_rsqrt(fvar));
                         const bool write = (run == 0) ? (tmod < R) : (tmod >= R);
@@ -1493,6 +1514,18 @@
         for (int cq = 0; cq < 2; ++cq)
             if (gx * 2 + cq < G16p) a.part_out[slot * G16p + gx * 2 + cq] = (cq == 0) ? tot : 0.0;
     }
+    if (MODE == MODE_FWD && a.sq_out) {
+#pragma unroll
+        for (int c = 0; c < 2; ++c)
+#pragma unroll
+            for (int qi = 0; qi < QPW; ++qi) {
+                double v2 = sq[c][qi];
+#pragma unroll
+                for (int o = 8; o > 0; o >>= 1) v2 += __shfl_xor(v2, o);
+                const int q = ((c == 0) ? w : (W - 1 - w)) + qi * W, d = 4 * q + g, grp = 2 * gx + c;
+                if (q < 4 && nl == 0 && d < a.dim_y && d < Do && grp < G16) a.sq_out[int64_t(grp) * a.dim_y + d] = v2;
+            }
+    }
 }
 
 }
diff --git a/cbf-ssm_amd/csrc/cbfssm_tail.hip b/cbf-ssm_amd/csrc/cbfssm_tail.hip
--- a/cbf-ssm_amd/csrc/cbfssm_tail.hip
+++ b/cbf-ssm_amd/csrc/cbfssm_tail.hip
@@ -325,6 +325,21 @@
     if (d == 0 && tid < 3) tail[tid] = out8[tid];
 }
 
+__global__ __launch_bounds__(256) void data_tail_sq_kernel(const double* sq_part, int64_t ngrp, int dim_y, const double* var_y,
+                                                           const double* out8, double cL, double bts, double* tail)
+{
+    __shared__ double red[4];
+    const int tid = threadIdx.x, d = blockIdx.x;
+    double s = 0.0;
+    for (int64_t k = tid; k < ngrp; k += 256) s += sq_part[k * dim_y + d];
+    const double sq = block_sum_t(s, red, tid, 256);
+    if (tid == 0) {
+        const double vy = var_y[d];
+        tail[3 + d] = -cL * 0.5 * (sq / (vy * vy) - bts / vy);
+    }
+    if (d == 0 && tid < 3) tail[tid] = out8[tid];
+}
+
 __global__ void adam_tick_kernel(double* t) { t[0] += 1.0; }
 
 __global__ __launch_bounds__(256) void adam_kernel(int64_t n, double* p, const double* g, double* m, double* v, const double* t,
@@ -553,6 +568,18 @@
     return e == hipSuccess ? 0 : fail(-int(e) - 1000, "data tail launch failed");
 }
 
+int cbfssm_data_tail_sq_f64(const cbfssm_problem* p, const double* var_y, const double* sq_part, const double* out8,
+                            double cL, double* tail, void* stream)
+{
+    if (!p || !var_y || !sq_part || !out8 || !tail) return fail(-1, "null pointer");
+    if (p->dim_y < 1) return fail(-1, "bad dim_y");
+    const int64_t ngrp = (int64_t(p->B) * p->S + 15) / 16;
+    hipLaunchKernelGGL(data_tail_sq_kernel, dim3(unsigned(p->dim_y)), dim3(256), 0, (hipStream_t)stream, sq_part, ngrp,
+                       p->dim_y, var_y, out8, cL, double(p->B) * p->T * p->S, tail);
+    hipError_t e = hipGetLastError();
+    return e == hipSuccess ? 0 : fail(-int(e) - 1000, "data tail launch failed");
+}
+
 int cbfssm_adam_step_f64(int64_t n, double* pflat, const double* gflat, double* m, double* v, double* t_dev, double lr,
                          double beta1, double beta2, double eps, void* stream)
 {
diff --git a/include/cbfssm_hip.h b/include/cbfssm_hip.h
--- a/include/cbfssm_hip.h
+++ b/include/cbfssm_hip.h
@@ -175,6 +175,16 @@
                             const double* ent_part, int64_t n_ent, const double* scal_f, const double* scal_b,
                             double* out, void* stream);
 
+int cbfssm_forward_pass_sq_f64(const cbfssm_problem* p, const cbfssm_pack_layout* layout_f, const double* pack_f,
+                               const double* var_x, const double* var_y, const double* u, const double* y,
+                               const double* y2, const double* eps_f, double* x, double* fmv_f, double* a2s_f,
+                               double* kl_part, double* sq_part, void* stream);
+int cbfssm_elbo_combine_sq_f64(const cbfssm_problem* p, double lambda0, double lambda1, const double* sq_part,
+                               const double* var_y, const double* kl_part, int64_t n_kl, const double* ent_part,
+                               int64_t n_ent, const double* scal_f, const double* scal_b, double* out, void* stream);
+int cbfssm_data_tail_sq_f64(const cbfssm_problem* p, const double* var_y, const double* sq_part, const double* out8,
+                            double cL, double* tail, void* stream);
+
 int64_t cbfssm_rev_workgroups(const cbfssm_problem* p, int backward_runs);
 
 int cbfssm_bwd_schedule(const cbfssm_problem* p, int cap, int* run, int* t_begin, int* nsteps);
@@ -222,6 +232,7 @@
 
 #define CBFSSM_REDUCE_SPLIT 32
 int cbfssm_reduce_partials_f64(double* gpart, int64_t slab, int64_t nwg, double* out, void* stream);
+
 
 int64_t cbfssm_stash_contract_work_elems(const cbfssm_pack_layout* layout, int64_t nslots);
 int cbfssm_stash_contract_f64(const cbfssm_pack_layout* layout, const double* stash_a, const double* stash_k, int64_t nslots,
```
